# SajayR/TRIAD

Measured on AMD Instinct MI355X. Metric: tri-modal triples/sec (whole node) + loss parity, B=256 at 1/2/4/8 MI355X, higher is better.
Workload: dtype bf16

## Files before the change

### include/triad_hip.h

```cpp
#ifndef TRIAD_HIP_H
#define TRIAD_HIP_H

#include <hip/hip_runtime_api.h>

#ifdef __cplusplus
extern "C" {
#endif

#define TRIAD_EINVAL 1001

int triad_pairsim_nparts(int R_pad, int Bk);

int triad_pairsim_fwd(const void* Q, const void* K, int R, int R_pad, int Nq, int Bq, int Bk, int Nk_pad,
                      int Nk_eff, int D, const float* temp, float clamp_lo, int diag, int diag_off,
                      float* rowmax, int* argmax, double* nn_part, float* diagS, void* dS, long long CT,
                      double* st_part, const int* k_len, hipStream_t stream);

typedef struct triad_pairsim_problem {
  const void* Q;
  const void* K;
  int R, R_pad, Nq, Bq, Bk, Nk_pad, Nk_eff;
  const float* temp;
  float clamp_lo;
  int diag, diag_off;
  float* rowmax;
  int* argmax;
  double* nn_part;
  float* diagS;
  void* dS;
  long long CT;
  double* st_part;
  const int* k_tiles;
} triad_pairsim_problem;

int triad_pairsim_fwd_multi(const triad_pairsim_problem* problems, int n, hipStream_t stream);

int triad_pairsim_diag(const triad_pairsim_problem* problems, int n, hipStream_t stream);

int triad_clip_reduce(const float* rowmax, int R_pad, int Nq, int Bq, int Bk, const float* qmask, float* clip,
                      float* qw, hipStream_t stream);

int triad_diag_smooth(const float* diagS, int Bq, int Nq, int Nk_pad, int Nk_eff, double cnt, double* part,
                      float* g, double* dt_part, hipStream_t stream);

int triad_diag_sparsity(const float* diagS, int Bq, int Nt, int Nk_pad, int Nk_eff, float thr, double cnt,
                        double* part, float* g, double* dt_part, hipStream_t stream);

int triad_losshead(const float* clip, int B, int kind, const float* temp, const double* nn_part, int n_nn,
                   double n_el, const double* dg_part, int n_dg, double dg_cnt, float w_sparse, float* out,
                   float* dclip, float* lse_scratch, hipStream_t stream);

int triad_pairsim_dS(const void* Q, const void* K, int R, int R_pad, int Nq, int Bq, int Bk, int Nk_pad,
                     int Nk_eff, int D, const float* temp, float clamp_lo, int diag, int diag_off,
                     const int* argmax, const float* dclip, const float* qw, const float* dSdiag,
                     const float* coef, void* dS, long long CT, double* dt_part, hipStream_t stream);

int triad_dS_patch(void* dS, long long CT, int R, int R_pad, int Nq, int Bq, int Bk, int Nk_pad, int Nk_eff,
                   int diag_off, const int* argmax, const float* rowmax, const float* dclip, const float* qw,
                   float ratio_max, const float* gdiag, float ratio_diag, double* max_part, int n_max_part,
                   const float* temp, hipStream_t stream);

int triad_dS_patch_tiles(void* dS, long long CT, int R, int R_pad, int Nq, int Bq, int Bk, int Nk_pad, int Nk_eff,
                         int diag_off, const int* argmax, const float* rowmax, const float* dclip, const float* qw,
                         float ratio_max, const float* gdiag, float ratio_diag, double* max_part, int n_max_part,
                         const float* temp, const int* k_tiles, hipStream_t stream);

int triad_dtemp_finalize(const double* p0, int n0, const double* p1, int n1, const double* p2, int n2,
                         const float* temp, const float* w, int has_cal, float* out, hipStream_t stream);

int triad_tile_gemm(const void* Dt, long long CT, int dk, const void* B, int M, int nkt, const float* alpha,
                    int splits, float* slabs, void* C, hipStream_t stream);

int triad_tile_gemm_slabs(const void* Dt, long long CT, int dk, const void* B, int M, int nkt, int splits,
                          float* slabs, hipStream_t stream);

int triad_bfrag_pack16(const void* B, int nkt, int dk, void* Bp, hipStream_t stream);
int triad_tile_gemm_packed16(const void* Dt, long long CT, int dk, const void* Bp, int M, int nkt, const float* alpha,
                             int splits, float* slabs, void* C, hipStream_t stream);
int triad_tile_gemm_packed16_slabs(const void* Dt, long long CT, int dk, const void* Bp, int M, int nkt, int splits,
                                   float* slabs, hipStream_t stream);

int triad_gemm_bf16(const void* A, long long lda, int a_kcontig, const void* B, long long ldb, int b_kcontig,
                    int M, int N, int Kd, const float* alpha, void* C, long long ldc, int out_bf16,
                    hipStream_t stream);

int triad_gemm_bf16_bias(const void* A, long long lda, int a_kcontig, const void* B, long long ldb, int b_kcontig,
                         int M, int N, int Kd, const float* bias, void* C, long long ldc, hipStream_t stream);

int triad_gemm_bf16_bias_bf16(const void* A, long long lda, int a_kcontig, const void* B, long long ldb,
                              int b_kcontig, int M, int N, int Kd, const void* bias, void* C, long long ldc,
                              hipStream_t stream);

int triad_gemm_bf16_splitk(const void* A, long long lda, int a_kcontig, const void* B, long long ldb, int b_kcontig,
                           int M, int N, int Kd, int splits, const float* alpha, float* slabs, void* C,
                           int out_bf16, hipStream_t stream);

int triad_gemm_bf16_splitk_form(const void* A, long long lda, int a_kcontig, const void* B, long long ldb,
                                int b_kcontig, int M, int N, int Kd, int splits, const float* alpha, float* slabs,
                                void* C, int out_bf16, int form, hipStream_t stream);

int triad_gemm_bf16_form(const void* A, long long lda, int a_kcontig, const void* B, long long ldb, int b_kcontig,
                         int M, int N, int Kd, const float* alpha, void* C, long long ldc, int out_bf16, int form,
                         hipStream_t stream);

int triad_wpack(const void* W, int K, void* Bp, hipStream_t stream);
int triad_wpack2(const void* W1, int K1, void* Bp1, const void* W2, int K2, void* Bp2, hipStream_t stream);
int triad_rowpanel_count(long long M);
int triad_projhead_fwd(const void* h, long long M, int H, long long lda, long long n_per, long long bstride,
                       const void* W1p, const void* b1, const float* gamma, const float* beta, float eps,
                       const void* W2p, const void* b2, void* y1, void* ln, float* mean, float* rstd, void* y,
                       hipStream_t stream);
int triad_projhead_ln_fwd(const void* h, long long M, int H, long long lda, long long n_per, long long bstride,
                          const void* W1p, const void* b1, const float* gamma, const float* beta, float eps, void* y1,
                          void* ln, float* mean, float* rstd, hipStream_t stream);
int triad_rowgemm_bias(const void* A, long long M, int K, long long lda, const void* Bp, const void* bias, void* C,
                       hipStream_t stream);
int triad_projhead_ln_bwd(const void* dy, long long M, const void* W2p, const void* y1, const float* mean,
                          const float* rstd, const float* gamma, void* dy1, float* part, hipStream_t stream);

int triad_similarity_maps(const void* f1, const void* f2, int B, int N1, int N2, int D, const float* temp, float eps,
                          float* sim, hipStream_t stream);

int triad_ln_fwd(const void* y1, int M, const float* gamma, const float* beta, float eps, void* ln, float* mean,
                 float* rstd, hipStream_t stream);

int triad_ln_bwd3(const void* dln, const void* y1, const float* mean, const float* rstd, const float* gamma, int M,
                  void* dy1, float* part, int nblocks, hipStream_t stream);

int triad_colsum_splits(long long rows, int cols);
int triad_colsum(const void* X, long long rows, int cols, long long ld, float* part, float alpha, int out_bf16,
                 void* out, hipStream_t stream);

int triad_colsum_dma_splits(long long rows, int cols);
int triad_colsum_dma(const void* X, long long rows, int cols, long long ld, float* part, float alpha, int out_bf16,
                     void* out, hipStream_t stream);

int triad_sum_slabs(const float* slabs, int nslab, long long n, const float* alpha, int out_bf16, void* out,
                    hipStream_t stream);

int triad_global_znorm(const float* x, long long n, float eps, float* y, double* part, int nblocks,
                       hipStream_t stream);

int triad_grad_sumsq(const float* g, const void* chunks, int nchunks, double* out, hipStream_t stream);
int triad_adamw_step(float* p, const float* g, float* m, float* v, const void* chunks, int nchunks,
                     const float* pp, const float* scale, float beta1, float beta2, float omb1, float omb2,
                     float eps, const unsigned long long* shadow, hipStream_t stream);
int triad_gather_grads(const void* pieces, int npieces, float* g, int accumulate, hipStream_t stream);

int triad_gather_rows(const void* src, long long src_rows, const int* idx, int B, int M, int row_bytes, void* dst,
                      hipStream_t stream);

int triad_l2norm_rows(const void* x, int rows, int D, float eps, void* y, hipStream_t stream);

int triad_retrieval_maxmean_f32(const float* Q, const int* qlen, int Bq, int nq_pad, const float* K, const int* klen,
                                int Bk, int nk_pad, int D, float temp, float* sim, hipStream_t stream);

int triad_l2norm_rows_f32(const float* x, int rows, int D, float eps, float* y, hipStream_t stream);

long long triad_chgn_workspace_bytes(int B, int T, int C);
int triad_chgn_gelu_fwd(const void* x, int B, int T, int Tp, int C, const float* gamma, const float* beta,
                        float eps, float* mean, float* rstd, void* ws, void* y, hipStream_t stream);
int triad_chgn_gelu_bwd(const void* x, const void* dy, int B, int T, int Tp, int C, const float* gamma,
                        const float* beta, const float* mean, const float* rstd, void* ws, void* dx, float* dgamma,
                        float* dbeta, hipStream_t stream);

int triad_c0gn_fwd(const void* wave, long long Lp, const void* w0, int B, int T, int Tp, int C, const float* gamma,
                   const float* beta, float eps, float* mean, float* rstd, void* ws, void* out, void* y0out,
                   hipStream_t stream);

long long triad_conv0_dw_workspace_bytes(int B, int T, int C);
int triad_conv0_dw(const void* wave, long long Lp, const void* dy0, int B, int T, int Tp, int C, void* ws, float* dw0,
                   hipStream_t stream);

int triad_posconv(const void* x, const void* wt, const float* bias, void* y, int B, int T, int C, int groups,
                  int pad, hipStream_t stream);

long long triad_posconv_dw_part_bytes(int C, int groups, int splits);
int triad_posconv_dw(const void* x, const void* dy, int B, int T, int C, int groups, int pad, int splits, float* part,
                     hipStream_t stream);

int triad_attn_fwd(const void* q, long long q_sB, long long q_sN, const void* k, long long k_sB, long long k_sN,
                   const void* v, long long v_sB, long long v_sN, int B, int H, int N, int D, float scale, void* out,
                   long long out_sB, long long out_sN, float* lse, hipStream_t stream);
int triad_attn_bwd(const void* q, long long q_sB, long long q_sN, const void* k, long long k_sB, long long k_sN,
                   const void* v, long long v_sB, long long v_sN, const void* o, long long o_sB, long long o_sN,
                   const void* dout, long long do_sB, long long do_sN, const float* lse, int B, int H, int N, int D,
                   float scale, void* dq, long long dq_sB, long long dq_sN, void* dk, long long dk_sB,
                   long long dk_sN, void* dv, long long dv_sB, long long dv_sN, float* delta, hipStream_t stream);
int triad_attn_dropmask(int B, int H, int N, float p, unsigned seed, unsigned* wq, unsigned* wk, hipStream_t stream);
int triad_attn_fwd_dropout(const void* q, long long q_sB, long long q_sN, const void* k, long long k_sB,
                           long long k_sN, const void* v, long long v_sB, long long v_sN, int B, int H, int N, int D,
                           float scale, const unsigned* wq, float p, void* out, long long out_sB, long long out_sN,
                           float* lse, hipStream_t stream);
int triad_attn_bwd_dropout(const void* q, long long q_sB, long long q_sN, const void* k, long long k_sB,
                           long long k_sN, const void* v, long long v_sB, long long v_sN, const void* o,
                           long long o_sB, long long o_sN, const void* dout, long long do_sB, long long do_sN,
                           const float* lse, int B, int H, int N, int D, float scale, const unsigned* wq,
                           const unsigned* wk, float p, void* dq, long long dq_sB, long long dq_sN, void* dk,
                           long long dk_sB, long long dk_sN, void* dv, long long dv_sB, long long dv_sN, float* delta,
                           hipStream_t stream);

int triad_rows_nt(const void* X, long long ldx, int M, int K, const void* W, int J, void* out, hipStream_t stream);
int triad_lora_update(void* Y, long long ldy, int M, int O, const void* T, const void* Bs, hipStream_t stream);
int triad_lora_tn_blocks(int M);
int triad_lora_tn(const void* Y, long long ldy, int M, int O, const void* T, const void* Wt, void* dt, float alpha,
                  float* slabs, float* out, hipStream_t stream);

int triad_addln_fwd(const float* x, const void* y, const float* g, const float* w, const float* b, float eps, int M,
                    int D, float* xn, void* ln, int out_f32, float* mean, float* rstd, hipStream_t stream);
int triad_addln_bwd(const void* dln, int dln_f32, const float* dres, const float* xn, const float* mean,
                    const float* rstd, const float* w, const float* g, int M, int D, float* dx, void* dy,
                    hipStream_t stream);

int triad_dropaddln_fwd(const float* res, const void* y, const float* w, const float* b, float eps, int M, int D,
                        float p, unsigned seed, float* h, void* hb, float* mean, float* rstd, hipStream_t stream);
int triad_dropaddln_bwd_blocks(int M);
int triad_dropaddln_bwd(const float* dh, const void* dhb, const float* res, const void* y, const float* mean,
                        const float* rstd, const float* w, int M, int D, float p, unsigned seed, float* dres, void* dy,
                        float* part, hipStream_t stream);
long long triad_gelu_table_bytes(void);
int triad_gelu_table(void* table, hipStream_t stream);
int triad_geludrop_fwd(const void* u, long long n, float p, unsigned seed, const void* table, void* v,
                       hipStream_t stream);
int triad_geludrop_bwd(const void* u, const void* dv, long long n, float p, unsigned seed, const void* table, void* du,
                       hipStream_t stream);
int triad_dropout_keep(long long n, float p, unsigned seed, void* out, hipStream_t stream);

int triad_dense_nparts(long long n);
int triad_dense_rowmax(const float* S, int Bq, int Bk, int Nq, int Nk, int R_pad, float* rowmax, int* argmax,
                       hipStream_t stream);
int triad_nonneg_fwd(const float* S, long long n, float lo, double* part, hipStream_t stream);
int triad_nonneg_bwd(const float* S, long long n, float lo, float scale, const float* coef, float* dS,
                     hipStream_t stream);
int triad_sims_bwd_pack(const float* S, const float* dtok, const float* dclip, const float* qw, const int* argmax,
                        int Bq, int Bk, int Nq, int Nk, int R_pad, const float* temp, void* A, long long lda,
                        double* part, hipStream_t stream);
int triad_sum_parts(const double* part, int n, double scale, float* out, hipStream_t stream);

#ifdef __cplusplus
}
#endif
#endif
```

### triad_amd/_lib.py

```python
from __future__ import annotations

import ctypes as C
import os
import threading

_HERE = os.path.dirname(os.path.abspath(__file__))
DEFAULT_LIB = os.path.join(_HERE, "libtriad_hip.so")
LIB_PATH = os.environ.get("TRIAD_LIB_VARIANT", DEFAULT_LIB)

vp, i32, u32, i64, f32, f64 = C.c_void_p, C.c_int, C.c_uint, C.c_longlong, C.c_float, C.c_double

SIGNATURES = {
    "triad_pairsim_nparts": [i32, i32],
    "triad_pairsim_fwd": [vp, vp, i32, i32, i32, i32, i32, i32, i32, i32, vp, f32, i32, i32, vp, vp, vp, vp, vp,
                          i64, vp, vp, vp],
    "triad_pairsim_fwd_multi": [vp, i32, vp],
    "triad_pairsim_diag": [vp, i32, vp],
    "triad_clip_reduce": [vp, i32, i32, i32, i32, vp, vp, vp, vp],
    "triad_diag_smooth": [vp, i32, i32, i32, i32, f64, vp, vp, vp, vp],
    "triad_diag_sparsity": [vp, i32, i32, i32, i32, f32, f64, vp, vp, vp, vp],
    "triad_losshead": [vp, i32, i32, vp, vp, i32, f64, vp, i32, f64, f32, vp, vp, vp, vp],
    "triad_pairsim_dS": [vp, vp, i32, i32, i32, i32, i32, i32, i32, i32, vp, f32, i32, i32, vp, vp, vp, vp, vp,
                         vp, i64, vp, vp],
    "triad_dS_patch": [vp, i64, i32, i32, i32, i32, i32, i32, i32, i32, vp, vp, vp, vp, f32, vp, f32, vp, i32, vp,
                       vp],
    "triad_dS_patch_tiles": [vp, i64, i32, i32, i32, i32, i32, i32, i32, i32, vp, vp, vp, vp, f32, vp, f32, vp, i32,
                             vp, vp, vp],
    "triad_dtemp_finalize": [vp, i32, vp, i32, vp, i32, vp, vp, i32, vp, vp],
    "triad_tile_gemm": [vp, i64, i32, vp, i32, i32, vp, i32, vp, vp, vp],
    "triad_tile_gemm_slabs": [vp, i64, i32, vp, i32, i32, i32, vp, vp],
    "triad_bfrag_pack16": [vp, i32, i32, vp, vp],
    "triad_tile_gemm_packed16": [vp, i64, i32, vp, i32, i32, vp, i32, vp, vp, vp],
    "triad_tile_gemm_packed16_slabs": [vp, i64, i32, vp, i32, i32, i32, vp, vp],
    "triad_gemm_bf16": [vp, i64, i32, vp, i64, i32, i32, i32, i32, vp, vp, i64, i32, vp],
    "triad_gemm_bf16_bias": [vp, i64, i32, vp, i64, i32, i32, i32, i32, vp, vp, i64, vp],
    "triad_gemm_bf16_bias_bf16": [vp, i64, i32, vp, i64, i32, i32, i32, i32, vp, vp, i64, vp],
    "triad_gemm_bf16_splitk": [vp, i64, i32, vp, i64, i32, i32, i32, i32, i32, vp, vp, vp, i32, vp],
    "triad_gemm_bf16_splitk_form": [vp, i64, i32, vp, i64, i32, i32, i32, i32, i32, vp, vp, vp, i32, i32, vp],
    "triad_wpack": [vp, i32, vp, vp],
    "triad_wpack2": [vp, i32, vp, vp, i32, vp, vp],
    "triad_projhead_fwd": [vp, i64, i32, i64, i64, i64, vp, vp, vp, vp, f32, vp, vp, vp, vp, vp, vp, vp, vp],
    "triad_similarity_maps": [vp, vp, i32, i32, i32, i32, vp, f32, vp, vp],
    "triad_rowpanel_count": [i64],
    "triad_projhead_ln_fwd": [vp, i64, i32, i64, i64, i64, vp, vp, vp, vp, f32, vp, vp, vp, vp, vp],
    "triad_rowgemm_bias": [vp, i64, i32, i64, vp, vp, vp, vp],
    "triad_projhead_ln_bwd": [vp, i64, vp, vp, vp, vp, vp, vp, vp, vp],
    "triad_ln_fwd": [vp, i32, vp, vp, f32, vp, vp, vp, vp],
    "triad_ln_bwd3": [vp, vp, vp, vp, vp, i32, vp, vp, i32, vp],
    "triad_sum_slabs": [vp, i32, i64, vp, i32, vp, vp],
    "triad_colsum_splits": [i64, i32],
    "triad_colsum": [vp, i64, i32, i64, vp, f32, i32, vp, vp],
    "triad_colsum_dma_splits": [i64, i32],
    "triad_colsum_dma": [vp, i64, i32, i64, vp, f32, i32, vp, vp],
    "triad_global_znorm": [vp, i64, f32, vp, vp, i32, vp],
    "triad_grad_sumsq": [vp, vp, i32, vp, vp],
    "triad_adamw_step": [vp, vp, vp, vp, vp, i32, vp, vp, f32, f32, f32, f32, f32, vp, vp],
    "triad_gather_grads": [vp, i32, vp, i32, vp],
    "triad_gather_rows": [vp, i64, vp, i32, i32, i32, vp, vp],
    "triad_l2norm_rows": [vp, i32, i32, f32, vp, vp],
    "triad_l2norm_rows_f32": [vp, i32, i32, f32, vp, vp],
    "triad_retrieval_maxmean_f32": [vp, vp, i32, i32, vp, vp, i32, i32, i32, f32, vp, vp],
    "triad_chgn_workspace_bytes": [i32, i32, i32],
    "triad_chgn_gelu_fwd": [vp, i32, i32, i32, i32, vp, vp, f32, vp, vp, vp, vp, vp],
    "triad_chgn_gelu_bwd": [vp, vp, i32, i32, i32, i32, vp, vp, vp, vp, vp, vp, vp, vp, vp],
    "triad_gemm_bf16_form": [vp, i64, i32, vp, i64, i32, i32, i32, i32, vp, vp, i64, i32, i32, vp],
    "triad_conv0_dw_workspace_bytes": [i32, i32, i32],
    "triad_conv0_dw": [vp, i64, vp, i32, i32, i32, i32, vp, vp, vp],
    "triad_c0gn_fwd": [vp, i64, vp, i32, i32, i32, i32, vp, vp, f32, vp, vp, vp, vp, vp, vp],
    "triad_posconv": [vp, vp, vp, vp, i32, i32, i32, i32, i32, vp],
    "triad_posconv_dw_part_bytes": [i32, i32, i32],
    "triad_posconv_dw": [vp, vp, i32, i32, i32, i32, i32, i32, vp, vp],
    "triad_rows_nt": [vp, i64, i32, i32, vp, i32, vp, vp],
    "triad_lora_update": [vp, i64, i32, i32, vp, vp, vp],
    "triad_dropaddln_fwd": [vp, vp, vp, vp, f32, i32, i32, f32, u32, vp, vp, vp, vp, vp],
    "triad_dropaddln_bwd_blocks": [i32],
    "triad_dropaddln_bwd": [vp, vp, vp, vp, vp, vp, vp, i32, i32, f32, u32, vp, vp, vp, vp],
    "triad_gelu_table_bytes": [],
    "triad_gelu_table": [vp, vp],
    "triad_geludrop_fwd": [vp, i64, f32, u32, vp, vp, vp],
    "triad_geludrop_bwd": [vp, vp, i64, f32, u32, vp, vp, vp],
    "triad_dropout_keep": [i64, f32, u32, vp, vp],
    "triad_addln_fwd": [vp, vp, vp, vp, vp, f32, i32, i32, vp, vp, i32, vp, vp, vp],
    "triad_addln_bwd": [vp, i32, vp, vp, vp, vp, vp, vp, i32, i32, vp, vp, vp],
    "triad_lora_tn_blocks": [i32],
    "triad_lora_tn": [vp, i64, i32, i32, vp, vp, vp, f32, vp, vp, vp],
    "triad_attn_dropmask": [i32, i32, i32, f32, u32, vp, vp, vp],
    "triad_attn_fwd_dropout": [vp, i64, i64, vp, i64, i64, vp, i64, i64, i32, i32, i32, i32, f32, vp, f32, vp, i64,
                               i64, vp, vp],
    "triad_attn_bwd_dropout": [vp, i64, i64, vp, i64, i64, vp, i64, i64, vp, i64, i64, vp, i64, i64, vp, i32, i32,
                               i32, i32, f32, vp, vp, f32, vp, i64, i64, vp, i64, i64, vp, i64, i64, vp, vp],
    "triad_attn_fwd": [vp, i64, i64, vp, i64, i64, vp, i64, i64, i32, i32, i32, i32, f32, vp, i64, i64, vp, vp],
    "triad_attn_bwd": [vp, i64, i64, vp, i64, i64, vp, i64, i64, vp, i64, i64, vp, i64, i64, vp, i32, i32, i32,
                       i32, f32, vp, i64, i64, vp, i64, i64, vp, i64, i64, vp, vp],
    "triad_dense_nparts": [i64],
    "triad_dense_rowmax": [vp, i32, i32, i32, i32, i32, vp, vp, vp],
    "triad_nonneg_fwd": [vp, i64, f32, vp, vp],
    "triad_nonneg_bwd": [vp, i64, f32, f32, vp, vp, vp],
    "triad_sims_bwd_pack": [vp, vp, vp, vp, vp, i32, i32, i32, i32, i32, vp, vp, i64, vp, vp],
    "triad_sum_parts": [vp, i32, f64, vp, vp],
}
RESTYPES = {"triad_pairsim_nparts": C.c_int, "triad_chgn_workspace_bytes": C.c_longlong,
            "triad_conv0_dw_workspace_bytes": C.c_longlong, "triad_gelu_table_bytes": C.c_longlong,
            "triad_posconv_dw_part_bytes": C.c_longlong,
            "triad_lora_tn_blocks": C.c_int, "triad_dropaddln_bwd_blocks": C.c_int,
            "triad_colsum_splits": C.c_int, "triad_colsum_dma_splits": C.c_int, "triad_dense_nparts": C.c_int,
            "triad_rowpanel_count": C.c_int}

BACKBONE_ENTRY_POINTS = frozenset({
    "triad_chgn_gelu_fwd", "triad_chgn_gelu_bwd", "triad_gemm_bf16_form", "triad_conv0_dw", "triad_c0gn_fwd",
    "triad_posconv", "triad_posconv_dw", "triad_gemm_bf16_splitk", "triad_rows_nt", "triad_lora_update",
    "triad_dropaddln_fwd", "triad_dropaddln_bwd", "triad_gelu_table", "triad_geludrop_fwd", "triad_geludrop_bwd",
    "triad_dropout_keep", "triad_addln_fwd", "triad_addln_bwd", "triad_lora_tn", "triad_attn_dropmask",
    "triad_attn_fwd_dropout", "triad_attn_bwd_dropout", "triad_attn_fwd", "triad_attn_bwd"})


def hot_path_entry_points():
    return tuple(n for n in SIGNATURES if n not in RESTYPES and n not in BACKBONE_ENTRY_POINTS)



class PairsimProblem(C.Structure):
    _fields_ = [("Q", vp), ("K", vp), ("R", i32), ("R_pad", i32), ("Nq", i32), ("Bq", i32), ("Bk", i32),
                ("Nk_pad", i32), ("Nk_eff", i32), ("temp", vp), ("clamp_lo", f32), ("diag", i32), ("diag_off", i32),
                ("rowmax", vp), ("argmax", vp), ("nn_part", vp), ("diagS", vp), ("dS", vp), ("CT", i64),
                ("st_part", vp), ("k_tiles", vp)]


_lock = threading.Lock()
_lib = None


class TriadError(RuntimeError):
    pass


def load():
    global _lib
    with _lock:
        if _lib is None:
            if not os.path.exists(LIB_PATH):
                raise TriadError(f"{LIB_PATH} not found: build it with `python -m triad_amd.build` "
                                 "(or __graft_entry__.build()); there is no CPU fallback")
            if LIB_PATH == DEFAULT_LIB:
                _check_fresh()
            lib = C.CDLL(LIB_PATH)
            for name, args in SIGNATURES.items():
                if LIB_PATH != DEFAULT_LIB and not hasattr(lib, name):
                    continue
                fn = getattr(lib, name)
                fn.argtypes = args
                fn.restype = RESTYPES.get(name, C.c_int)
            _lib = lib
    return _lib


def _check_fresh():
    from . import build
    stamp = DEFAULT_LIB + ".srchash"
    have = open(stamp).read().strip() if os.path.exists(stamp) else None
    if have != build.source_hash():
        raise TriadError(f"{DEFAULT_LIB} is stale (built from different sources than triad_amd/csrc + "
                         "include): rebuild with `python -m triad_amd.build`")


TIMERS = None
WATCH = None


def _isolate(name):
    spec = os.environ.get("TRIAD_ISOLATE")
    return bool(spec) and name not in RESTYPES and any(name.startswith(p) for p in spec.split(",") if p)


def call(name, *args, meta=None):
    if _isolate(name):
        import torch
        torch.cuda.synchronize()
        try:
            rc = getattr(load(), name)(*args)
        finally:
            torch.cuda.synchronize()
    elif TIMERS is not None and name in TIMERS:
        import torch
        e0, e1 = torch.cuda.Event(enable_timing=True), torch.cuda.Event(enable_timing=True)
        e0.record()
        rc = getattr(load(), name)(*args)
        e1.record()
        TIMERS[name].append((e0, e1, meta))
    else:
        rc = getattr(load(), name)(*args)
    if WATCH is not None and name not in RESTYPES:
        WATCH.note(name)
    if name not in RESTYPES and rc != 0:
        what = "invalid argument/shape" if rc == 1001 else f"hipError_t {rc}"
        raise TriadError(f"{name} failed: {what}")
    return rc


def ptr(t):
    return None if t is None else C.c_void_p(t.data_ptr())


def h2d(t, device):
    import torch
    device = torch.device(device)
    if device.type != "cuda":
        return t.to(device)
    return t.pin_memory().to(device, non_blocking=True)


def stream_ptr(device=None):
    import torch
    return C.c_void_p(torch.cuda.current_stream(device).cuda_stream)
```

### triad_amd/csrc/gemm.hip

```cpp
#include "common.h"

namespace {

constexpr int BM = 128, BN = 128, BK = 64;
constexpr int A_ELEMS = BM * BK, B_ELEMS = BK * BN;

__device__ __forceinline__ int kc_off(int m, int chunk) { return m * BK + ((chunk ^ ((m >> 1) & 7)) << 3); }
__device__ __forceinline__ int nc_off(int k, int col) {
  return k * BN + ((((col >> 3) ^ ((k & 3) << 2))) << 3) + (col & 7);
}

template <bool A_KCONTIG>
__device__ __forceinline__ void stage_a_piece(const bf16* __restrict__ A, long long lda, int m0, int k0, bf16* dst,
                                              int wave, int lane, int u) {
  const int inst = wave * 4 + u;
  if (A_KCONTIG) {
    const int m = inst * 8 + (lane >> 3), cp = lane & 7;
    const int c = cp ^ ((m >> 1) & 7);
    glds16(A + (size_t)(m0 + m) * lda + k0 + c * 8, dst + inst * 512);
  } else {
    const int k = inst * 4 + (lane >> 4), cp = lane & 15;
    const int c = cp ^ ((k & 3) << 2);
    glds16(A + (size_t)(k0 + k) * lda + m0 + c * 8, dst + inst * 512);
  }
}

template <bool A_KCONTIG>
__device__ __forceinline__ void stage_a(const bf16* __restrict__ A, long long lda, int m0, int k0, bf16* dst,
                                        int wave, int lane) {
#pragma unroll
  for (int u = 0; u < 4; ++u) stage_a_piece<A_KCONTIG>(A, lda, m0, k0, dst, wave, lane, u);
}


template <bool B_KCONTIG>
__device__ __forceinline__ void stage_b(const bf16* __restrict__ B, long long ldb, int n0, int k0, bf16* dst,
                                        int wave, int lane) {
  stage_a<B_KCONTIG>(B, ldb, n0, k0, dst, wave, lane);
}

__device__ __forceinline__ bf16x8 frag_tr(const bf16* img, int n0, int s, int lane) {
  const int g = lane >> 4, i = lane & 15, q = i >> 2, p = i & 3, hh = g >> 1;
  const int col = n0 + 16 * (g & 1) + 4 * p;
  const int k0 = 16 * s + 8 * hh + q;
  const s16x4 lo = lds_tr16(img + nc_off(k0, col));
  const s16x4 hi = lds_tr16(img + nc_off(k0 + 4, col));
  bf16x8 r;
  s16x4* rp = (s16x4*)&r;
  rp[0] = lo;
  rp[1] = hi;
  return r;
}

__device__ __forceinline__ float bias_at(const void* bias, int bias_bf16, int n) {
  if (!bias) return 0.f;
  return bias_bf16 ? (float)((const bf16*)bias)[n] : ((const float*)bias)[n];
}

__device__ __forceinline__ void tile_split(int xsplit, int& tile, int& split) {
  const int T = gridDim.x;
  if (xsplit) {
    const int L = blockIdx.y * T + blockIdx.x, c = L % 8, i = L / 8;
    tile = i % T;
    split = c + 8 * (i / T);
    return;
  }
  const int bid = blockIdx.x, q8 = T / 8, r8 = T % 8, x = bid % 8;
  tile = (x < r8 ? x * (q8 + 1) : r8 * (q8 + 1) + (x - r8) * q8) + bid / 8;
  split = blockIdx.y;
}

template <bool A_KCONTIG, bool B_KCONTIG, typename OutT>
__global__ __launch_bounds__(256, 2) void gemm_kernel(const bf16* __restrict__ A, long long lda,
                                                      const bf16* __restrict__ B, long long ldb,
                                                      int M, int N, int Kd, const float* __restrict__ alpha_p,
                                                      OutT* __restrict__ C, long long ldc, int k_per_split,
                                                      long long slab_stride, const void* __restrict__ bias, int bias_bf16, int xsplit) {
  __shared__ __attribute__((aligned(16))) bf16 lds[2 * (A_ELEMS + B_ELEMS)];
  const int lane = threadIdx.x & 63, wave = __builtin_amdgcn_readfirstlane(threadIdx.x >> 6);
  const int wm = wave >> 1, wn = wave & 1;
  const int h = lane >> 5;

  int swz, split;
  tile_split(xsplit, swz, split);
  const int ntn = N / BN;
  const int m0 = (swz / ntn) * BM, n0 = (swz % ntn) * BN;

  f32x16 acc[2][2];
#pragma unroll
  for (int a = 0; a < 2; ++a)
#pragma unroll
    for (int b = 0; b < 2; ++b) acc[a][b] = (f32x16){};

  const int kbeg = split * k_per_split;
  const int nk = min(k_per_split, Kd - kbeg) / BK;
  C += (size_t)split * slab_stride;
  if (nk > 0) {
    stage_a<A_KCONTIG>(A, lda, m0, kbeg, lds, wave, lane);
    stage_b<B_KCONTIG>(B, ldb, n0, kbeg, lds + A_ELEMS, wave, lane);
  }
  for (int kt = 0; kt < nk; ++kt) {
    lds_dma_barrier();
    bf16* const nb = lds + ((kt + 1) & 1) * (A_ELEMS + B_ELEMS);
    const bool pf = kt + 1 < nk;
    if (pf) {
      stage_a<A_KCONTIG>(A, lda, m0, kbeg + (kt + 1) * BK, nb, wave, lane);
      stage_b<B_KCONTIG>(B, ldb, n0, kbeg + (kt + 1) * BK, nb + A_ELEMS, wave, lane);
    }
    const bf16* ai = lds + (kt & 1) * (A_ELEMS + B_ELEMS);
    const bf16* bi = ai + A_ELEMS;
#pragma unroll
    for (int s = 0; s < BK / 16; ++s) {
      bf16x8 af[2], bfr[2];
#pragma unroll
      for (int t = 0; t < 2; ++t) {
        const int mrow = wm * 64 + t * 32;
        if (A_KCONTIG) {
          af[t] = *(const bf16x8*)(ai + kc_off(mrow + (lane & 31), 2 * s + h));
        } else {
          af[t] = frag_tr(ai, mrow, s, lane);
        }
        const int ncol = wn * 64 + t * 32;
        if (B_KCONTIG) {
          bfr[t] = *(const bf16x8*)(bi + kc_off(ncol + (lane & 31), 2 * s + h));
        } else {
          bfr[t] = frag_tr(bi, ncol, s, lane);
        }
      }
#pragma unroll
      for (int a = 0; a < 2; ++a)
#pragma unroll
        for (int b = 0; b < 2; ++b) {
          acc[a][b] = mfma32(af[a], bfr[b], acc[a][b]);
        }
    }
  }

  const float alpha = alpha_p ? *alpha_p : 1.f;
#pragma unroll
  for (int a = 0; a < 2; ++a)
#pragma unroll
    for (int b = 0; b < 2; ++b) {
      const int n = n0 + wn * 64 + b * 32 + (lane & 31);
      const float bn = bias_at(bias, bias_bf16, n);
#pragma unroll
      for (int v = 0; v < 16; ++v) {
        const int m = m0 + wm * 64 + a * 32 + (v & 3) + 8 * (v >> 2) + 4 * h;
        C[(size_t)m * ldc + n] = (OutT)(alpha * acc[a][b][v] + bn);
      }
    }
}

constexpr int GB_M = 256, GB_NB = 3;
constexpr int GB_A = GB_M * BK, GB_ST = GB_A + B_ELEMS;
constexpr int GB_PIECES = 6;


template <bool A_KCONTIG, bool B_KCONTIG>
__device__ __forceinline__ void gb_piece(const bf16* __restrict__ A, long long lda, const bf16* __restrict__ B,
                                         long long ldb, int m0, int n0, int k0, bf16* dst, int wave, int lane,
                                         int u) {
  if (u < 4) {
    const int inst = wave * 4 + u;
    if (A_KCONTIG) {
      const int m = inst * 8 + (lane >> 3), cp = lane & 7;
      const int c = cp ^ ((m >> 1) & 7);
      glds16(A + (size_t)(m0 + m) * lda + k0 + c * 8, dst + inst * 512);
    } else {
      const int half = inst >> 4, ii = inst & 15;
      const int k = ii * 4 + (lane >> 4), cp = lane & 15;
      const int c = cp ^ ((k & 3) << 2);
      glds16(A + (size_t)(k0 + k) * lda + m0 + half * 128 + c * 8, dst + half * (BK * 128) + ii * 512);
    }
  } else {
    const int inst = wave * 2 + (u - 4);
    bf16* bd = dst + GB_A;
    if (B_KCONTIG) {
      const int n = inst * 8 + (lane >> 3), cp = lane & 7;
      const int c = cp ^ ((n >> 1) & 7);
      glds16(B + (size_t)(n0 + n) * ldb + k0 + c * 8, bd + inst * 512);
    } else {
      const int k = inst * 4 + (lane >> 4), cp = lane & 15;
      const int c = cp ^ ((k & 3) << 2);
      glds16(B + (size_t)(k0 + k) * ldb + n0 + c * 8, bd + inst * 512);
    }
  }
}

template <bool A_KCONTIG, bool B_KCONTIG, typename OutT>
__global__ __launch_bounds__(512, 1) void gemm_big_kernel(const bf16* __restrict__ A, long long lda,
                                                          const bf16* __restrict__ B, long long ldb, int M, int N,
                                                          int Kd, const float* __restrict__ alpha_p,
                                                          OutT* __restrict__ C, long long ldc, int k_per_split,
                                                          long long slab_stride, const void* __restrict__ bias, int bias_bf16, int xsplit) {
  __shared__ __attribute__((aligned(16))) bf16 lds[GB_NB * GB_ST];
  const int lane = threadIdx.x & 63, wave = __builtin_amdgcn_readfirstlane(threadIdx.x >> 6);
  const int wm = wave >> 1, wn = wave & 1;
  const int h = lane >> 5;
  int swz, split;
  tile_split(xsplit, swz, split);
  const int ntn = N / BN;
  const int m0 = (swz / ntn) * GB_M, n0 = (swz % ntn) * BN;

  f32x16 acc[2][2];
#pragma unroll
  for (int a = 0; a < 2; ++a)
#pragma unroll
    for (int b = 0; b < 2; ++b) acc[a][b] = (f32x16){};

  const int kbeg = split * k_per_split;
  const int nk = __builtin_amdgcn_readfirstlane(max(0, min(k_per_split, Kd - kbeg)) / BK);
  C += (size_t)split * slab_stride;
#pragma unroll
  for (int p = 0; p < GB_NB - 1; ++p)
    if (p < nk)
#pragma unroll
      for (int u = 0; u < GB_PIECES; ++u)
        gb_piece<A_KCONTIG, B_KCONTIG>(A, lda, B, ldb, m0, n0, kbeg + p * BK, lds + p * GB_ST, wave, lane, u);
  for (int kt = 0; kt < nk; ++kt) {
    if (kt + 1 < nk) TRIAD_VMCNT(GB_PIECES);
    else asm volatile("s_waitcnt vmcnt(0)" ::: "memory");
    __syncthreads();
    const bool pf = kt + GB_NB - 1 < nk;
    bf16* const nb = lds + ((kt + GB_NB - 1) % GB_NB) * GB_ST;
    const int kn = kbeg + (kt + GB_NB - 1) * BK;
    const bf16* ai = lds + (kt % GB_NB) * GB_ST;
    const bf16* bi = ai + GB_A;
#pragma unroll
    for (int s = 0; s < BK / 16; ++s) {
      bf16x8 af[2], bfr[2];
#pragma unroll
      for (int t = 0; t < 2; ++t) {
        const int mrow = wm * 64 + t * 32;
        if (A_KCONTIG) af[t] = *(const bf16x8*)(ai + kc_off(mrow + (lane & 31), 2 * s + h));
        else af[t] = frag_tr(ai + (mrow >> 7) * (BK * 128), mrow & 127, s, lane);
        const int ncol = wn * 64 + t * 32;
        if (B_KCONTIG) bfr[t] = *(const bf16x8*)(bi + kc_off(ncol + (lane & 31), 2 * s + h));
        else bfr[t] = frag_tr(bi, ncol, s, lane);
      }
#pragma unroll
      for (int a = 0; a < 2; ++a)
#pragma unroll
        for (int b = 0; b < 2; ++b) {
          acc[a][b] = mfma32(af[a], bfr[b], acc[a][b]);
          const int mi = s * 4 + a * 2 + b;
          if ((mi & 1) && mi / 2 < GB_PIECES) {
            __builtin_amdgcn_sched_barrier(0);
            if (pf) gb_piece<A_KCONTIG, B_KCONTIG>(A, lda, B, ldb, m0, n0, kn, nb, wave, lane, mi / 2);
            __builtin_amdgcn_sched_barrier(0);
          }
        }
    }
  }

  const float alpha = alpha_p ? *alpha_p : 1.f;
#pragma unroll
  for (int a = 0; a < 2; ++a)
#pragma unroll
    for (int b = 0; b < 2; ++b) {
      const int n = n0 + wn * 64 + b * 32 + (lane & 31);
      const float bn = bias_at(bias, bias_bf16, n);
#pragma unroll
      for (int v = 0; v < 16; ++v) {
        const int m = m0 + wm * 64 + a * 32 + (v & 3) + 8 * (v >> 2) + 4 * h;
        C[(size_t)m * ldc + n] = (OutT)(alpha * acc[a][b][v] + bn);
      }
    }
}

constexpr int GW_M = 256, GW_N = 256;
constexpr int GW_A = GW_M * BK, GW_ST = GW_A + GW_N * BK;

template <bool KCONTIG>
__device__ __forceinline__ void gw_piece_one(const bf16* __restrict__ X, long long ld, int r0, int k0, bf16* img,
                                             int inst, int lane) {
  if (KCONTIG) {
    const int m = inst * 8 + (lane >> 3), cp = lane & 7;
    const int c = cp ^ ((m >> 1) & 7);
    glds16(X + (size_t)(r0 + m) * ld + k0 + c * 8, img + inst * 512);
  } else {
    const int half = inst >> 4, ii = inst & 15;
    const int k = ii * 4 + (lane >> 4), cp = lane & 15;
    const int c = cp ^ ((k & 3) << 2);
    glds16(X + (size_t)(k0 + k) * ld + r0 + half * 128 + c * 8, img + half * (BK * 128) + ii * 512);
  }
}

template <bool KCONTIG>
__device__ __forceinline__ bf16x8 gw_frag(const bf16* img, int row, int s, int lane) {
  if (KCONTIG) return *(const bf16x8*)(img + kc_off(row + (lane & 31), 2 * s + (lane >> 5)));
  return frag_tr(img + (row >> 7) * (BK * 128), row & 127, s, lane);
}

constexpr int GE_PIECES = 8;

template <bool A_KCONTIG, bool B_KCONTIG>
__device__ __forceinline__ void ge_piece(const bf16* __restrict__ A, long long lda, const bf16* __restrict__ B,
                                         long long ldb, int m0, int n0, int k0, bf16* dst, int wave, int lane,
                                         int u) {
  if (u < 4) gw_piece_one<A_KCONTIG>(A, lda, m0, k0, dst, wave * 4 + u, lane);
  else gw_piece_one<B_KCONTIG>(B, ldb, n0, k0, dst + GW_A, wave * 4 + (u - 4), lane);
}

template <bool A_KCONTIG, bool B_KCONTIG, typename OutT>
__global__ __launch_bounds__(512, 1) void gemm_w8_kernel(const bf16* __restrict__ A, long long lda,
                                                         const bf16* __restrict__ B, long long ldb, int M, int N,
                                                         int Kd, const float* __restrict__ alpha_p,
                                                         OutT* __restrict__ C, long long ldc, int k_per_split,
                                                         long long slab_stride, const void* __restrict__ bias, int bias_bf16, int xsplit) {
  __shared__ __attribute__((aligned(16))) bf16 lds[2 * GW_ST];
  const int lane = threadIdx.x & 63, wave = __builtin_amdgcn_readfirstlane(threadIdx.x >> 6);
  const int wm = wave >> 2, wn = wave & 3;
  const int h = lane >> 5;
  int swz, split;
  tile_split(xsplit, swz, split);
  const int ntn = N / GW_N;
  const int m0 = (swz / ntn) * GW_M, n0 = (swz % ntn) * GW_N;

  f32x16 acc[4][2];
#pragma unroll
  for (int a = 0; a < 4; ++a)
#pragma unroll
    for (int b = 0; b < 2; ++b) acc[a][b] = (f32x16){};

  const int kbeg = split * k_per_split;
  const int nk = __builtin_amdgcn_readfirstlane(max(0, min(k_per_split, Kd - kbeg)) / BK);
  C += (size_t)split * slab_stride;
  if (nk > 0)
#pragma unroll
    for (int u = 0; u < GE_PIECES; ++u)
      ge_piece<A_KCONTIG, B_KCONTIG>(A, lda, B, ldb, m0, n0, kbeg, lds, wave, lane, u);
  for (int kt = 0; kt < nk; ++kt) {
    asm volatile("s_waitcnt vmcnt(0)" ::: "memory");
    __syncthreads();
    const bool pf = kt + 1 < nk;
    bf16* const nb = lds + ((kt + 1) & 1) * GW_ST;
    const int kn = kbeg + (kt + 1) * BK;
    const bf16* ai = lds + (kt & 1) * GW_ST;
    const bf16* bi = ai + GW_A;
    bf16x8 af[2][4], bfr[2][2];
#pragma unroll
    for (int t = 0; t < 4; ++t) af[0][t] = gw_frag<A_KCONTIG>(ai, wm * 128 + t * 32, 0, lane);
#pragma unroll
    for (int t = 0; t < 2; ++t) bfr[0][t] = gw_frag<B_KCONTIG>(bi, wn * 64 + t * 32, 0, lane);
#pragma unroll
    for (int s = 0; s < BK / 16; ++s) {
      const int cur = s & 1;
#pragma unroll
      for (int a = 0; a < 4; ++a)
#pragma unroll
        for (int b = 0; b < 2; ++b) {
          acc[a][b] = mfma32(af[cur][a], bfr[cur][b], acc[a][b]);
          const int j = a * 2 + b, mi = s * 8 + j;
          if (s + 1 < BK / 16 && j < 6) {
            __builtin_amdgcn_sched_barrier(0);
            if (j < 4) af[cur ^ 1][j] = gw_frag<A_KCONTIG>(ai, wm * 128 + j * 32, s + 1, lane);
            else bfr[cur ^ 1][j - 4] = gw_frag<B_KCONTIG>(bi, wn * 64 + (j - 4) * 32, s + 1, lane);
            __builtin_amdgcn_sched_barrier(0);
          }
          if (mi % 2 == 1 && mi / 2 < GE_PIECES) {
            __builtin_amdgcn_sched_barrier(0);
            if (pf) ge_piece<A_KCONTIG, B_KCONTIG>(A, lda, B, ldb, m0, n0, kn, nb, wave, lane, mi / 2);
            __builtin_amdgcn_sched_barrier(0);
          }
        }
    }
  }

  const float alpha = alpha_p ? *alpha_p : 1.f;
#pragma unroll
  for (int a = 0; a < 4; ++a)
#pragma unroll
    for (int b = 0; b < 2; ++b) {
      const int n = n0 + wn * 64 + b * 32 + (lane & 31);
      const float bn = bias_at(bias, bias_bf16, n);
#pragma unroll
      for (int v = 0; v < 16; ++v) {
        const int m = m0 + wm * 128 + a * 32 + (v & 3) + 8 * (v >> 2) + 4 * h;
        C[(size_t)m * ldc + n] = (OutT)(alpha * acc[a][b][v] + bn);
      }
    }
}


constexpr int kBigForm = 4;
constexpr int kXcdSplit = 8;


template <bool AK, bool BK_, typename OutT>
int launch(const void* A, long long lda, const void* B, long long ldb, int M, int N, int Kd, const float* alpha,
           void* C, long long ldc, hipStream_t st, int splits = 1, long long slab_stride = 0,
           const void* bias = nullptr, int form = 0, int bias_bf16 = 0) {
  const int xsplit = (form & kXcdSplit) ? 1 : 0;
  form &= ~kXcdSplit;
  if (M % BM || N % BN || Kd % BK || lda % 8 || ldb % 8 || splits < 1) return TRIAD_EINVAL;
  if (xsplit && splits % 8) return TRIAD_EINVAL;
  const int kps = ((Kd / BK + splits - 1) / splits) * BK;
  const bool w4_ok = M % GW_M == 0 && N % GW_N == 0;
  const bool w4_auto = AK && BK_ && splits == 1 && M >= 65536 && Kd >= 1024;
  if (form == 0 && w4_ok && w4_auto) form = kBigForm;
  if (w4_ok && (form == 4 || form == 3)) {
    const int nwg = (M / GW_M) * (N / GW_N);
    hipLaunchKernelGGL((gemm_w8_kernel<AK, BK_, OutT>), dim3(nwg, splits), dim3(512), 0, st, (const bf16*)A, lda,
                       (const bf16*)B, ldb, M, N, Kd, alpha, (OutT*)C, ldc, kps, slab_stride, bias, bias_bf16, xsplit);
    TRIAD_CHECK_LAUNCH();
    return TRIAD_OK;
  }
  if (form != 1 && M % GB_M == 0 &&
      (form == 2 || M >= 8192 || Kd / splits >= 32768)) {
    const int nwg = (M / GB_M) * (N / BN);
    hipLaunchKernelGGL((gemm_big_kernel<AK, BK_, OutT>), dim3(nwg, splits), dim3(512), 0, st, (const bf16*)A, lda,
                       (const bf16*)B, ldb, M, N, Kd, alpha, (OutT*)C, ldc, kps, slab_stride, bias, bias_bf16, xsplit);
    TRIAD_CHECK_LAUNCH();
    return TRIAD_OK;
  }
  const int nwg = (M / BM) * (N / BN);
  hipLaunchKernelGGL((gemm_kernel<AK, BK_, OutT>), dim3(nwg, splits), dim3(256), 0, st, (const bf16*)A, lda,
                     (const bf16*)B, ldb, M, N, Kd, alpha, (OutT*)C, ldc, kps, slab_stride, bias, bias_bf16, xsplit);
  TRIAD_CHECK_LAUNCH();
  return TRIAD_OK;
}

}

extern "C" {

int triad_gemm_bf16_form(const void* A, long long lda, int a_kcontig, const void* B, long long ldb, int b_kcontig,
                         int M, int N, int Kd, const float* alpha, void* C, long long ldc, int out_bf16, int form,
                         hipStream_t stream) {
  if (form < 0 || form > 4) return TRIAD_EINVAL;
#define TRIAD_GEMM_CASE(AK, BKC)                                                                  \
  if (!!a_kcontig == AK && !!b_kcontig == BKC)                                                   \
    return out_bf16 ? launch<AK, BKC, bf16>(A, lda, B, ldb, M, N, Kd, alpha, C, ldc, stream, 1, 0, nullptr, form) \
                    : launch<AK, BKC, float>(A, lda, B, ldb, M, N, Kd, alpha, C, ldc, stream, 1, 0, nullptr, form);
  TRIAD_GEMM_CASE(true, true)
  TRIAD_GEMM_CASE(true, false)
  TRIAD_GEMM_CASE(false, true)
  TRIAD_GEMM_CASE(false, false)
#undef TRIAD_GEMM_CASE
  return TRIAD_EINVAL;
}

int triad_gemm_bf16(const void* A, long long lda, int a_kcontig, const void* B, long long ldb, int b_kcontig,
                    int M, int N, int Kd, const float* alpha, void* C, long long ldc, int out_bf16,
                    hipStream_t stream) {
  return triad_gemm_bf16_form(A, lda, a_kcontig, B, ldb, b_kcontig, M, N, Kd, alpha, C, ldc, out_bf16, 0, stream);
}

static int gemm_bias_launch(const void* A, long long lda, int a_kcontig, const void* B, long long ldb, int b_kcontig, int M,
                     int N, int Kd, const void* bias, int bias_bf16, void* C, long long ldc, hipStream_t stream) {
  int form = 1;
  if (M >= 32768 && M % GW_M == 0 && N % GW_N == 0) form = kBigForm;
  else if (M >= 8192 && M % GB_M == 0 && (long long)(M / GB_M) * (N / BN) >= 256) form = 2;
#define TRIAD_GEMM_B(AK, BKC)                                                                     \
  if (!!a_kcontig == AK && !!b_kcontig == BKC)                                                    \
    return launch<AK, BKC, bf16>(A, lda, B, ldb, M, N, Kd, nullptr, C, ldc, stream, 1, 0, bias, form, bias_bf16);
  TRIAD_GEMM_B(true, true)
  TRIAD_GEMM_B(true, false)
  TRIAD_GEMM_B(false, true)
  TRIAD_GEMM_B(false, false)
#undef TRIAD_GEMM_B
  return TRIAD_EINVAL;
}

int triad_gemm_bf16_bias(const void* A, long long lda, int a_kcontig, const void* B, long long ldb, int b_kcontig,
                         int M, int N, int Kd, const float* bias, void* C, long long ldc, hipStream_t stream) {
  return gemm_bias_launch(A, lda, a_kcontig, B, ldb, b_kcontig, M, N, Kd, bias, 0, C, ldc, stream);
}

int triad_gemm_bf16_bias_bf16(const void* A, long long lda, int a_kcontig, const void* B, long long ldb,
                              int b_kcontig, int M, int N, int Kd, const void* bias, void* C, long long ldc,
                              hipStream_t stream) {
  return gemm_bias_launch(A, lda, a_kcontig, B, ldb, b_kcontig, M, N, Kd, bias, 1, C, ldc, stream);
}

int triad_gemm_bf16_splitk_form(const void* A, long long lda, int a_kcontig, const void* B, long long ldb,
                                int b_kcontig, int M, int N, int Kd, int splits, const float* alpha, float* slabs,
                                void* C, int out_bf16, int form, hipStream_t stream) {
  if ((form & ~kXcdSplit) < 0 || (form & ~kXcdSplit) > 4) return TRIAD_EINVAL;
  const long long slab = (long long)M * N;
  int rc = TRIAD_EINVAL;
#define TRIAD_GEMM_SK(AK, BKC)                                                                  \
  if (!!a_kcontig == AK && !!b_kcontig == BKC)                                                 \
    rc = launch<AK, BKC, float>(A, lda, B, ldb, M, N, Kd, nullptr, slabs, N, stream, splits, slab, nullptr, form);
  TRIAD_GEMM_SK(true, true)
  TRIAD_GEMM_SK(true, false)
  TRIAD_GEMM_SK(false, true)
  TRIAD_GEMM_SK(false, false)
#undef TRIAD_GEMM_SK
  if (rc) return rc;
  return triad_sum_slabs(slabs, splits, slab, alpha, out_bf16, C, stream);
}

int triad_gemm_bf16_splitk(const void* A, long long lda, int a_kcontig, const void* B, long long ldb, int b_kcontig,
                           int M, int N, int Kd, int splits, const float* alpha, float* slabs, void* C,
                           int out_bf16, hipStream_t stream) {
  return triad_gemm_bf16_splitk_form(A, lda, a_kcontig, B, ldb, b_kcontig, M, N, Kd, splits, alpha, slabs, C,
                                     out_bf16, 0, stream);
}

}
```

### triad_amd/gemm.py

```python
from __future__ import annotations

import torch
import torch.nn.functional as F

from ._lib import call, ptr, stream_ptr

_BF = torch.bfloat16
def _ok(M, N, K):
    return M > 0 and M % 128 == 0 and N % 128 == 0 and K % 64 == 0


def _rows(x):
    x2 = x.reshape(-1, x.shape[-1])
    if x2.stride(1) != 1 or x2.stride(0) != x2.shape[1]:
        x2 = x2.contiguous()
    return x2


def linear(x: torch.Tensor, w: torch.Tensor, b: torch.Tensor | None = None, meta=None) -> torch.Tensor:
    xb = x if x.dtype == _BF else x.to(_BF)
    wb = w if w.dtype == _BF else w.to(_BF)
    K = xb.shape[-1]
    N = wb.shape[0]
    x2 = _rows(xb)
    M = x2.shape[0]
    if not (x2.is_cuda and _ok(M, N, K)):
        return F.linear(xb, wb, None if b is None else b.to(_BF))
    wc = wb if wb.is_contiguous() else wb.contiguous()
    bias = None if b is None else b.detach().to(_BF).contiguous()
    out = torch.empty(M, N, dtype=_BF, device=x2.device)
    call("triad_gemm_bf16_bias_bf16", ptr(x2), K, 1, ptr(wc), K, 1, M, N, K, ptr(bias), ptr(out), N,
         stream_ptr(x2.device), meta=meta or dict(backbone=True, flops=2.0 * M * N * K))
    return out.view(*xb.shape[:-1], N)


def mm(a: torch.Tensor, b: torch.Tensor, meta=None) -> torch.Tensor:
    ab = a if a.dtype == _BF else a.to(_BF)
    bb = b if b.dtype == _BF else b.to(_BF)
    M, K = ab.shape
    N = bb.shape[1]
    if not (ab.is_cuda and _ok(M, N, K)):
        return ab @ bb
    a2 = ab if ab.is_contiguous() else ab.contiguous()
    b2 = bb if bb.is_contiguous() else bb.contiguous()
    out = torch.empty(M, N, dtype=_BF, device=a2.device)
    call("triad_gemm_bf16_bias", ptr(a2), K, 1, ptr(b2), N, 0, M, N, K, None, ptr(out), N, stream_ptr(a2.device),
         meta=meta or dict(backbone=True, flops=2.0 * M * N * K))
    return out
```

### triad_amd/linear.py

```python
from __future__ import annotations

import os

import torch
import torch.nn as nn
import torch.nn.functional as F

from . import _lib
from . import gemm as hipgemm
from ._lib import call, ptr, stream_ptr



_SPLITS_LONG = {36: 7, 108: 9, 144: 7}
_SPLITS_SHORT = {36: 7, 108: 4, 144: 3}


def _splits(M, out_f, in_f):
    tiles = (out_f // 128) * (in_f // 128)
    table = _SPLITS_LONG if M >= 32768 else _SPLITS_SHORT if 4096 <= M < 16384 else {}
    if tiles in table:
        return table[tiles]
    return min(8 if tiles <= 160 else 4, max(2, M // 2048))


_W8_SPLITS = {27: 8, 9: 24, 36: 12}
_W8_XCD = {27, 9}


def _form_splits(M, out_f, in_f):
    tiles8 = (out_f // 256) * (in_f // 256) if out_f % 256 == 0 and in_f % 256 == 0 else 0
    if M >= 32768 and tiles8 in _W8_SPLITS:
        return 4 | (8 if tiles8 in _W8_XCD else 0), _W8_SPLITS[tiles8]
    return 0, _splits(M, out_f, in_f)


def weight_grad(dy2: torch.Tensor, x2: torch.Tensor) -> torch.Tensor:
    M, O = dy2.shape
    K = x2.shape[1]
    if M % 64:
        Mp = (M + 63) // 64 * 64
        dy2 = torch.cat([dy2, dy2.new_zeros(Mp - M, O)])
        x2 = torch.cat([x2, x2.new_zeros(Mp - M, K)])
        M = Mp
    form, sp = _form_splits(M, O, K)
    slabs = torch.empty(sp * O * K, dtype=torch.float32, device=dy2.device)
    dw = torch.empty(O, K, dtype=torch.bfloat16, device=dy2.device)
    call("triad_gemm_bf16_splitk_form", ptr(dy2), dy2.stride(0), 0, ptr(x2), x2.stride(0), 0, O, K, M, sp, None,
         ptr(slabs), ptr(dw), 1, form, stream_ptr(dy2.device), meta=dict(backbone=True))
    return dw


_SIDE = {}
_JOIN_TASK = {}


def _dev_index(dev) -> int:
    dev = torch.device(dev)
    return dev.index if dev.index is not None else torch.cuda.current_device()


def _side_stream(dev):
    i = _dev_index(dev)
    s = _SIDE.get(i)
    if s is None:
        s = _SIDE[i] = torch.cuda.Stream(device=i)
    return s


def _join(dev):
    def cb():
        torch.cuda.current_stream(dev).wait_stream(_side_stream(dev))
    return cb


_CLAIMED = {}


def side_stream_ok(*ws: torch.Tensor) -> bool:
    task = torch._C._current_graph_task_id()
    if not (SIDE_STREAM_DW and task != -1 and all(w.is_cuda and w.dtype == torch.bfloat16 and w.grad is None
                                                   for w in ws)):
        return False
    dev = ws[0].device
    di = _dev_index(dev)
    t, seen = _CLAIMED.get(di, (None, None))
    if t != task:
        seen = set()
        _CLAIMED[di] = (task, seen)
    if any(id(w) in seen for w in ws):
        if di in _SIDE:
            torch.cuda.current_stream(dev).wait_stream(_SIDE[di])
        seen.update(id(w) for w in ws)
        return False
    seen.update(id(w) for w in ws)
    return True


def on_side_stream(fn, inputs):
    dev = inputs[0].device
    main = torch.cuda.current_stream(dev)
    side = _side_stream(dev)
    side.wait_stream(main)
    with torch.cuda.stream(side):
        outs = fn()
    for t in inputs:
        t.record_stream(side)
    for o in (outs if isinstance(outs, (list, tuple)) else (outs,)):
        o.record_stream(main)
    task = torch._C._current_graph_task_id()
    if _JOIN_TASK.get(_dev_index(dev)) != task:
        _JOIN_TASK[_dev_index(dev)] = task
        torch.autograd.Variable._execution_engine.queue_callback(_join(dev))
    return outs


SIDE_STREAM_DW = os.environ.get("TRIAD_SIDE_STREAM_DW", "1") != "0"


class _LinearFn(torch.autograd.Function):
    @staticmethod
    def forward(ctx, x, w, b):
        xb = x.to(torch.bfloat16)
        wb = w.to(torch.bfloat16)
        bb = None if b is None else b.to(torch.bfloat16)
        ctx.save_for_backward(xb, wb)
        ctx.meta = (x.dtype, w.dtype, None if b is None else b.dtype)
        ctx.w_ref = w
        return hipgemm.linear(xb, wb, bb)

    @staticmethod
    def backward(ctx, dy):
        xb, wb = ctx.saved_tensors
        x_dtype, w_dtype, b_dtype = ctx.meta
        O, K = wb.shape
        dy2 = dy.reshape(-1, O).to(torch.bfloat16).contiguous()
        x2 = xb.reshape(-1, K)
        if x2.stride(1) != 1 or x2.stride(0) != K:
            x2 = x2.contiguous()
        dx = dw = db = None
        if ctx.needs_input_grad[0]:
            dx = hipgemm.mm(dy2, wb).view(*xb.shape).to(x_dtype)
        if ctx.needs_input_grad[1]:
            if w_dtype == torch.bfloat16 and side_stream_ok(ctx.w_ref):
                dw = on_side_stream(lambda: weight_grad(dy2, x2), (dy2, x2))
            else:
                dw = weight_grad(dy2, x2).to(w_dtype)
        if b_dtype is not None and ctx.needs_input_grad[2]:
            from .ops import bias_grad
            db = bias_grad(dy2, torch.bfloat16 if b_dtype == torch.bfloat16 else torch.float32).to(b_dtype)
        return dx, dw, db


class _QKVFn(torch.autograd.Function):

    @staticmethod
    def forward(ctx, x, wq, bq, wk, bk, wv, bv):
        xb = x.to(torch.bfloat16)
        wb = torch.cat([wq, wk, wv]).to(torch.bfloat16)
        bb = None if bq is None else torch.cat([bq, bk, bv]).to(torch.bfloat16)
        ctx.save_for_backward(xb, wb)
        ctx.meta = (x.dtype, wq.dtype, None if bq is None else bq.dtype, (wq.shape[0], wk.shape[0], wv.shape[0]))
        ctx.w_refs = (wq, wk, wv)
        return hipgemm.linear(xb, wb, bb)

    @staticmethod
    def backward(ctx, dy):
        xb, wb = ctx.saved_tensors
        x_dtype, w_dtype, b_dtype, sizes = ctx.meta
        O, K = wb.shape
        dy2 = dy.reshape(-1, O).to(torch.bfloat16).contiguous()
        x2 = xb.reshape(-1, K)
        if x2.stride(1) != 1 or x2.stride(0) != K:
            x2 = x2.contiguous()
        dx = hipgemm.mm(dy2, wb).view(*xb.shape).to(x_dtype) if ctx.needs_input_grad[0] else None
        dws = [None] * 3
        if any(ctx.needs_input_grad[i] for i in (1, 3, 5)):
            if w_dtype == torch.bfloat16 and side_stream_ok(*ctx.w_refs):
                dws = list(on_side_stream(lambda: _split_rows(weight_grad(dy2, x2), sizes), (dy2, x2)))
            else:
                dws = [t.to(w_dtype) for t in weight_grad(dy2, x2).split(sizes)]
        dbs = [None] * 3
        if b_dtype is not None and any(ctx.needs_input_grad[i] for i in (2, 4, 6)):
            from .ops import bias_grad
            db = bias_grad(dy2, torch.bfloat16 if b_dtype == torch.bfloat16 else torch.float32).to(b_dtype)
            dbs = list(db.split(sizes))
        return dx, dws[0], dbs[0], dws[1], dbs[1], dws[2], dbs[2]


def _split_rows(buf: torch.Tensor, sizes):
    out, r = [], 0
    K = buf.shape[1]
    for n in sizes:
        t = torch.empty((0,), dtype=buf.dtype, device=buf.device)
        t.set_(buf.untyped_storage(), buf.storage_offset() + r * K, (n, K), (K, 1))
        out.append(t)
        r += n
    return out


def qkv_eligible(q: nn.Linear, k: nn.Linear, v: nn.Linear, x: torch.Tensor) -> bool:
    return (all(_eligible(m, x) for m in (q, k, v)) and q.in_features == k.in_features == v.in_features
            and (q.bias is None) == (k.bias is None) == (v.bias is None))


def qkv_projection(q: nn.Linear, k: nn.Linear, v: nn.Linear, x: torch.Tensor) -> torch.Tensor:
    return _QKVFn.apply(x, q.weight, q.bias, k.weight, k.bias, v.weight, v.bias)


def _eligible(mod: nn.Linear, x: torch.Tensor) -> bool:
    if not (x.is_cuda and torch.is_autocast_enabled("cuda") and torch.get_autocast_dtype("cuda") == torch.bfloat16):
        return False
    return x.numel() > 0 and mod.in_features % 128 == 0 and mod.out_features % 128 == 0


class TriadLinear(nn.Linear):

    def forward(self, x):
        if _eligible(self, x):
            return _LinearFn.apply(x, self.weight, self.bias)
        return super().forward(x)


def install_fast_linear(root: nn.Module) -> nn.Module:
    for mod in root.modules():
        if type(mod) is nn.Linear:
            mod.__class__ = TriadLinear
    return root
```

### triad_amd/vit.py

```python
from __future__ import annotations

import math

import torch
import torch.nn as nn
import torch.nn.functional as F

from . import attention
from . import gemm as hipgemm
from ._lib import call, ptr, stream_ptr
from .frontend import patch_embed
from .postln import gelu

ARCHS = {
    "dinov2_vits14_reg": (384, 12, 6),
    "dinov2_vitb14_reg": (768, 12, 12),
    "dinov2_vitl14_reg": (1024, 24, 16),
    "dinov2_vits14": (384, 12, 6),
    "dinov2_vitb14": (768, 12, 12),
    "dinov2_vitl14": (1024, 24, 16),
}


class _LoRALinear(torch.autograd.Function):

    @staticmethod
    def forward(ctx, x, w, b, A, B, scaling):
        lead, K = x.shape[:-1], x.shape[-1]
        O, r = B.shape
        xb = x.reshape(-1, K).to(torch.bfloat16).contiguous()
        M = xb.shape[0]
        dev = x.device
        st = stream_ptr(dev)
        Ab = A.detach().to(torch.bfloat16).contiguous()
        sB = (B.detach() * scaling).to(torch.bfloat16).contiguous()
        y = hipgemm.linear(xb, w.to(torch.bfloat16), None if b is None else b.to(torch.bfloat16)).contiguous()
        t = torch.empty(M, r, dtype=torch.bfloat16, device=dev)
        call("triad_rows_nt", ptr(xb), K, M, K, ptr(Ab), r, ptr(t), st)
        call("triad_lora_update", ptr(y), O, M, O, ptr(t), ptr(sB), st)
        ctx.save_for_backward(xb, w, Ab, sB, t)
        ctx.meta = (lead, x.dtype, float(scaling), A.dtype, B.dtype)
        return y.view(*lead, O)

    @staticmethod
    def backward(ctx, dy):
        xb, w, Ab, sB, t = ctx.saved_tensors
        lead, x_dtype, scaling, a_dtype, b_dtype = ctx.meta
        M, K = xb.shape
        O, r = sB.shape
        dev = xb.device
        dy2 = dy.reshape(M, O).to(torch.bfloat16).contiguous()
        st = stream_ptr(dev)
        dt = torch.empty(M, r, dtype=torch.bfloat16, device=dev)
        G = call("triad_lora_tn_blocks", M)
        slabs = torch.empty(G * max(O, K) * r, dtype=torch.float32, device=dev)
        wt = torch.zeros(16, O, dtype=torch.bfloat16, device=dev)
        wt[:r].copy_(sB.t())
        dB = torch.empty(O, r, dtype=torch.float32, device=dev)
        call("triad_lora_tn", ptr(dy2), O, M, O, ptr(t), ptr(wt), ptr(dt), scaling, ptr(slabs), ptr(dB), st)
        dx = None
        if ctx.needs_input_grad[0]:
            dx = hipgemm.mm(dy2, w.to(torch.bfloat16))
            At = Ab.t().contiguous()
            call("triad_lora_update", ptr(dx), K, M, K, ptr(dt), ptr(At), st)
            dx = dx.view(*lead, K).to(x_dtype)
        dAt = torch.empty(K, r, dtype=torch.float32, device=dev)
        call("triad_lora_tn", ptr(xb), K, M, K, ptr(dt), None, None, 1.0, ptr(slabs), ptr(dAt), st)
        return dx, None, None, dAt.t().to(a_dtype), dB.to(b_dtype), None


def lora_linear(x, w, b, A, B, scaling):
    return _LoRALinear.apply(x, w, b, A, B, scaling)


class LoRALinear(nn.Module):

    def __init__(self, base: nn.Linear, r: int = 8, alpha: int = 16):
        super().__init__()
        self.base = base
        self.lora_A = nn.Parameter(torch.empty(r, base.in_features))
        self.lora_B = nn.Parameter(torch.zeros(base.out_features, r))
        nn.init.kaiming_uniform_(self.lora_A, a=math.sqrt(5))
        self.scaling = alpha / r

    @property
    def weight(self):
        return self.base.weight

    def forward(self, x):
        if x.is_cuda and torch.is_autocast_enabled("cuda") and not self.base.weight.requires_grad \
                and (self.base.bias is None or not self.base.bias.requires_grad) and self.lora_A.shape[0] == 8 \
                and self.lora_A.shape[1] % 256 == 0 and self.lora_B.shape[0] % 256 == 0:
            return lora_linear(x, self.base.weight, self.base.bias, self.lora_A, self.lora_B, self.scaling)
        return self.base(x) + F.linear(F.linear(x, self.lora_A), self.lora_B) * self.scaling


class Attention(nn.Module):
    def __init__(self, dim, heads):
        super().__init__()
        self.heads = heads
        self.qkv = nn.Linear(dim, 3 * dim, bias=True)
        self.proj = nn.Linear(dim, dim, bias=True)

    def forward(self, x):
        B, N, C = x.shape
        qkv = self.qkv(x)
        if attention.supported(qkv, N, C // self.heads):
            return self.proj(attention.attention_qkv(qkv, self.heads))
        qkv = qkv.reshape(B, N, 3, self.heads, C // self.heads).permute(2, 0, 3, 1, 4)
        o = F.scaled_dot_product_attention(qkv[0], qkv[1], qkv[2])
        return self.proj(o.transpose(1, 2).reshape(B, N, C))


class LayerScale(nn.Module):
    def __init__(self, dim, init=1e-5):
        super().__init__()
        self.gamma = nn.Parameter(torch.full((dim,), init))

    def forward(self, x):
        return x * self.gamma


class Mlp(nn.Module):
    def __init__(self, dim, hidden):
        super().__init__()
        self.fc1 = nn.Linear(dim, hidden)
        self.fc2 = nn.Linear(hidden, dim)

    def forward(self, x):
        return self.fc2(gelu(self.fc1(x)))


class _AddScaleLN(torch.autograd.Function):

    @staticmethod
    def forward(ctx, x, y, g, w, b, eps, out_f32):
        M, D = x.numel() // x.shape[-1], x.shape[-1]
        dev = x.device
        if not (x.dtype == torch.float32 and y.dtype == torch.bfloat16 and y.shape == x.shape
                and all(p.dtype == torch.float32 and p.numel() == D for p in (g, w, b))):
            raise TypeError(f"add_scale_ln: x {x.dtype} {tuple(x.shape)}, y {y.dtype} {tuple(y.shape)}")
        x = x.contiguous()
        y = y.contiguous()
        xn = torch.empty_like(x)
        ln = torch.empty(x.shape, dtype=torch.float32 if out_f32 else torch.bfloat16, device=dev)
        mean = torch.empty(M, dtype=torch.float32, device=dev)
        rstd = torch.empty(M, dtype=torch.float32, device=dev)
        call("triad_addln_fwd", ptr(x), ptr(y), ptr(g), ptr(w), ptr(b), eps, M, D, ptr(xn), ptr(ln), int(out_f32),
             ptr(mean), ptr(rstd), stream_ptr(dev))
        ctx.save_for_backward(xn, mean, rstd, w, g)
        return xn, ln

    @staticmethod
    def backward(ctx, dxn, dln):
        xn, mean, rstd, w, g = ctx.saved_tensors
        M, D = xn.numel() // xn.shape[-1], xn.shape[-1]
        dev = xn.device
        if dln is None:
            dln = torch.zeros_like(xn)
        dln = dln.contiguous()
        if dln.shape != xn.shape or dln.dtype not in (torch.float32, torch.bfloat16) or \
                (dxn is not None and (dxn.shape != xn.shape or dxn.dtype != torch.float32)):
            raise TypeError("add_scale_ln backward: unexpected gradient layout")
        dxn = None if dxn is None else dxn.contiguous()
        dx = torch.empty_like(xn)
        dy = torch.empty(xn.shape, dtype=torch.bfloat16, device=dev)
        call("triad_addln_bwd", ptr(dln), int(dln.dtype == torch.float32), ptr(dxn), ptr(xn), ptr(mean), ptr(rstd),
             ptr(w), ptr(g), M, D, ptr(dx), ptr(dy), stream_ptr(dev))
        return dx, dy, None, None, None, None, None


def add_scale_ln(x, y, ls, norm, out_f32=False):
    return _AddScaleLN.apply(x, y, ls.gamma, norm.weight, norm.bias, norm.eps, out_f32)


class Block(nn.Module):
    def __init__(self, dim, heads, mlp_ratio=4.0, ls_init=1e-5):
        super().__init__()
        self.norm1 = nn.LayerNorm(dim, eps=1e-6)
        self.attn = Attention(dim, heads)
        self.ls1 = LayerScale(dim, ls_init)
        self.norm2 = nn.LayerNorm(dim, eps=1e-6)
        self.mlp = Mlp(dim, int(dim * mlp_ratio))
        self.ls2 = LayerScale(dim, ls_init)

    def forward(self, x):
        x = x + self.ls1(self.attn(self.norm1(x)))
        return x + self.ls2(self.mlp(self.norm2(x)))


class PatchEmbed(nn.Module):
    def __init__(self, patch, dim):
        super().__init__()
        self.proj = nn.Conv2d(3, dim, kernel_size=patch, stride=patch)

    def forward(self, x):
        return patch_embed(x, self.proj.weight, self.proj.bias, self.proj.stride[0])


class DinoVisionTransformer(nn.Module):

    def __init__(self, arch="dinov2_vitb14_reg", img_size=518, patch=14):
        super().__init__()
        dim, depth, heads = ARCHS[arch]
        self.embed_dim = dim
        self.patch_size = patch
        self.num_register_tokens = 4 if arch.endswith("_reg") else 0
        self.interpolate_antialias = self.num_register_tokens > 0
        self.interpolate_offset = 0.0 if self.num_register_tokens > 0 else 0.1
        grid = img_size // patch
        self.patch_embed = PatchEmbed(patch, dim)
        self.cls_token = nn.Parameter(torch.zeros(1, 1, dim))
        self.pos_embed = nn.Parameter(torch.zeros(1, 1 + grid * grid, dim))
        self.register_tokens = (nn.Parameter(torch.zeros(1, self.num_register_tokens, dim))
                                if self.num_register_tokens else None)
        self.mask_token = nn.Parameter(torch.zeros(1, dim))
        self.blocks = nn.ModuleList([Block(dim, heads) for _ in range(depth)])
        self.norm = nn.LayerNorm(dim, eps=1e-6)
        nn.init.trunc_normal_(self.pos_embed, std=0.02)
        nn.init.normal_(self.cls_token, std=1e-6)
        if self.register_tokens is not None:
            nn.init.normal_(self.register_tokens, std=1e-6)
        self.apply(self._init)
        self._pos_cache = {}

    @staticmethod
    def _init(m):
        if isinstance(m, nn.Linear):
            nn.init.trunc_normal_(m.weight, std=0.02)
            if m.bias is not None:
                nn.init.zeros_(m.bias)

    def refresh_frozen_copies(self):
        self._pos_cache = {}

    def interpolate_pos_encoding(self, n_patches_h, n_patches_w, dtype):
        key = (n_patches_h, n_patches_w, dtype, self.pos_embed._version)
        if not self.pos_embed.requires_grad and key in self._pos_cache:
            return self._pos_cache[key]
        pos = self.pos_embed.float()
        cls_pos, patch_pos = pos[:, :1], pos[:, 1:]
        M = int(math.sqrt(patch_pos.shape[1]))
        if (n_patches_h, n_patches_w) != (M, M):
            patch_pos = F.interpolate(patch_pos.reshape(1, M, M, -1).permute(0, 3, 1, 2),
                                      size=(n_patches_h, n_patches_w), mode="bicubic",
                                      antialias=self.interpolate_antialias)
            patch_pos = patch_pos.permute(0, 2, 3, 1).reshape(1, -1, pos.shape[-1])
        out = torch.cat([cls_pos, patch_pos], dim=1).to(dtype)
        if not self.pos_embed.requires_grad:
            self._pos_cache = {key: out.detach()}
        return out

    def prepare_tokens(self, x):
        B, _, H, W = x.shape
        t = self.patch_embed(x)
        t = torch.cat([self.cls_token.expand(B, -1, -1).to(t.dtype), t], dim=1)
        t = t + self.interpolate_pos_encoding(H // self.patch_size, W // self.patch_size, t.dtype)
        if self.register_tokens is not None:
            t = torch.cat([t[:, :1], self.register_tokens.expand(B, -1, -1).to(t.dtype), t[:, 1:]], dim=1)
        return t

    def _fused_ok(self, t, n, norm):
        return (t.is_cuda and n == 1 and norm and torch.is_autocast_enabled("cuda")
                and torch.get_autocast_dtype("cuda") == torch.bfloat16 and self.embed_dim % 256 == 0
                and self.embed_dim <= 1536
                and not any(p.requires_grad for blk in self.blocks
                            for m in (blk.norm1, blk.norm2, blk.ls1, blk.ls2) for p in m.parameters())
                and not any(p.requires_grad for p in self.norm.parameters()))

    def _blocks_fused(self, t):
        t = t.float()
        ln = F.layer_norm(t, (self.embed_dim,), self.blocks[0].norm1.weight, self.blocks[0].norm1.bias,
                          self.blocks[0].norm1.eps)
        last = len(self.blocks) - 1
        for i, blk in enumerate(self.blocks):
            t, ln = add_scale_ln(t, blk.attn(ln), blk.ls1, blk.norm2)
            nxt = self.norm if i == last else self.blocks[i + 1].norm1
            t, ln = add_scale_ln(t, blk.mlp(ln), blk.ls2, nxt, out_f32=i == last)
        return ln

    def get_intermediate_layers(self, x, n=1, norm=True):
        t = self.prepare_tokens(x)
        if self._fused_ok(t, n, norm):
            return (self._blocks_fused(t)[:, 1 + self.num_register_tokens:],)
        outs = []
        start = len(self.blocks) - n
        for i, blk in enumerate(self.blocks):
            t = blk(t)
            if i >= start:
                outs.append(t)
        if norm:
            outs = [self.norm(o) for o in outs]
        skip = 1 + self.num_register_tokens
        return tuple(o[:, skip:] for o in outs)

    def forward(self, x):
        t = self.prepare_tokens(x)
        for blk in self.blocks:
            t = blk(t)
        return self.norm(t)[:, 0]


def apply_lora(vit: DinoVisionTransformer, r=8, alpha=16, targets=("attn.qkv", "attn.proj")):
    for p in vit.parameters():
        p.requires_grad = False
    for blk in vit.blocks:
        if "attn.qkv" in targets:
            blk.attn.qkv = LoRALinear(blk.attn.qkv, r, alpha)
        if "attn.proj" in targets:
            blk.attn.proj = LoRALinear(blk.attn.proj, r, alpha)
    for n, p in vit.named_parameters():
        p.requires_grad = "lora_" in n
    return vit


def store_frozen_base_bf16(vit: nn.Module):
    masters = {}
    for mname, mod in vit.named_modules():
        if isinstance(mod, (nn.Linear, nn.Conv2d)):
            for pname, p in mod.named_parameters(recurse=False):
                if not p.requires_grad and p.dtype != torch.bfloat16:
                    masters[f"{mname}.{pname}" if mname else pname] = p.data.detach().to("cpu", torch.float32,
                                                                                            copy=True)
                    p.data = p.data.to(torch.bfloat16)
    vit.frozen_fp32 = {**getattr(vit, "frozen_fp32", {}), **masters}
    return vit
```

Measured before the change: 1964.

## Fuse LoRA rank-8 update into GEMM tail and bias grad into weight-grad GEMM

```diff
diff --git a/include/triad_hip.h b/include/triad_hip.h
--- a/include/triad_hip.h
+++ b/include/triad_hip.h
@@ -96,6 +96,14 @@
                            int out_bf16, hipStream_t stream);
 
 int triad_gemm_bf16_splitk_form(const void* A, long long lda, int a_kcontig, const void* B, long long ldb,
+                                int b_kcontig, int M, int N, int Kd, int splits, const float* alpha, float* slabs,
+                                void* C, int out_bf16, int form, hipStream_t stream);
+
+int triad_gemm_bf16_bias_rank8(const void* A, long long lda, int a_kcontig, const void* B, long long ldb,
+                               int b_kcontig, int M, int N, int Kd, const void* T, const void* U, const void* bias,
+                               void* C, long long ldc, int form, hipStream_t stream);
+
+int triad_gemm_bf16_splitk_bias(const void* A, long long lda, int a_kcontig, const void* B, long long ldb,
                                 int b_kcontig, int M, int N, int Kd, int splits, const float* alpha, float* slabs,
                                 void* C, int out_bf16, int form, hipStream_t stream);
 
diff --git a/triad_amd/_lib.py b/triad_amd/_lib.py
--- a/triad_amd/_lib.py
+++ b/triad_amd/_lib.py
@@ -37,6 +37,8 @@
     "triad_gemm_bf16_bias_bf16": [vp, i64, i32, vp, i64, i32, i32, i32, i32, vp, vp, i64, vp],
     "triad_gemm_bf16_splitk": [vp, i64, i32, vp, i64, i32, i32, i32, i32, i32, vp, vp, vp, i32, vp],
     "triad_gemm_bf16_splitk_form": [vp, i64, i32, vp, i64, i32, i32, i32, i32, i32, vp, vp, vp, i32, i32, vp],
+    "triad_gemm_bf16_bias_rank8": [vp, i64, i32, vp, i64, i32, i32, i32, i32, vp, vp, vp, vp, i64, i32, vp],
+    "triad_gemm_bf16_splitk_bias": [vp, i64, i32, vp, i64, i32, i32, i32, i32, i32, vp, vp, vp, i32, i32, vp],
     "triad_wpack": [vp, i32, vp, vp],
     "triad_wpack2": [vp, i32, vp, vp, i32, vp, vp],
     "triad_projhead_fwd": [vp, i64, i32, i64, i64, i64, vp, vp, vp, vp, f32, vp, vp, vp, vp, vp, vp, vp, vp],
@@ -108,7 +110,8 @@
 
 BACKBONE_ENTRY_POINTS = frozenset({
     "triad_chgn_gelu_fwd", "triad_chgn_gelu_bwd", "triad_gemm_bf16_form", "triad_conv0_dw", "triad_c0gn_fwd",
-    "triad_posconv", "triad_posconv_dw", "triad_gemm_bf16_splitk", "triad_rows_nt", "triad_lora_update",
+    "triad_posconv", "triad_posconv_dw", "triad_gemm_bf16_splitk", "triad_gemm_bf16_splitk_bias", "triad_rows_nt",
+    "triad_lora_update",
     "triad_dropaddln_fwd", "triad_dropaddln_bwd", "triad_gelu_table", "triad_geludrop_fwd", "triad_geludrop_bwd",
     "triad_dropout_keep", "triad_addln_fwd", "triad_addln_bwd", "triad_lora_tn", "triad_attn_dropmask",
     "triad_attn_fwd_dropout", "triad_attn_bwd_dropout", "triad_attn_fwd", "triad_attn_bwd"})
@@ -143,6 +146,7 @@
                                  "(or __graft_entry__.build()); there is no CPU fallback")
             if LIB_PATH == DEFAULT_LIB:
                 _check_fresh()
+            import torch
             lib = C.CDLL(LIB_PATH)
             for name, args in SIGNATURES.items():
                 if LIB_PATH != DEFAULT_LIB and not hasattr(lib, name):
diff --git a/triad_amd/csrc/gemm.hip b/triad_amd/csrc/gemm.hip
--- a/triad_amd/csrc/gemm.hip
+++ b/triad_amd/csrc/gemm.hip
@@ -57,6 +57,20 @@
   return bias_bf16 ? (float)((const bf16*)bias)[n] : ((const float*)bias)[n];
 }
 
+__device__ __forceinline__ bf16x8 r8_load(const bf16* __restrict__ X, int row, int lane) {
+  return *(const bf16x8*)(X + (size_t)(row + (lane & 31)) * 8);
+}
+__device__ __forceinline__ bf16x8 r8_frag(bf16x8 v, int lane) { return (lane >> 5) ? (bf16x8){} : v; }
+
+typedef __bf16 bf16x2 __attribute__((ext_vector_type(2)));
+__device__ __forceinline__ float frag_ksum(bf16x8 a, float c) {
+  const bf16x2 one = {(bf16)1.f, (bf16)1.f};
+  const bf16x2* p = (const bf16x2*)&a;
+#pragma unroll
+  for (int j = 0; j < 4; ++j) c = __builtin_amdgcn_fdot2_f32_bf16(p[j], one, c, false);
+  return c;
+}
+
 __device__ __forceinline__ void tile_split(int xsplit, int& tile, int& split) {
   const int T = gridDim.x;
   if (xsplit) {
@@ -70,12 +84,13 @@
   split = blockIdx.y;
 }
 
-template <bool A_KCONTIG, bool B_KCONTIG, typename OutT>
+template <bool A_KCONTIG, bool B_KCONTIG, typename OutT, bool COLSUM = false>
 __global__ __launch_bounds__(256, 2) void gemm_kernel(const bf16* __restrict__ A, long long lda,
                                                       const bf16* __restrict__ B, long long ldb,
                                                       int M, int N, int Kd, const float* __restrict__ alpha_p,
                                                       OutT* __restrict__ C, long long ldc, int k_per_split,
-                                                      long long slab_stride, const void* __restrict__ bias, int bias_bf16, int xsplit) {
+                                                      long long slab_stride, const void* __restrict__ bias, int bias_bf16, int xsplit,
+                                                      const bf16* __restrict__ T, const bf16* __restrict__ U) {
   __shared__ __attribute__((aligned(16))) bf16 lds[2 * (A_ELEMS + B_ELEMS)];
   const int lane = threadIdx.x & 63, wave = __builtin_amdgcn_readfirstlane(threadIdx.x >> 6);
   const int wm = wave >> 1, wn = wave & 1;
@@ -95,6 +110,17 @@
   const int kbeg = split * k_per_split;
   const int nk = min(k_per_split, Kd - kbeg) / BK;
   C += (size_t)split * slab_stride;
+  bf16x8 tf[2] = {}, uf[2] = {};
+  const bool tail = !COLSUM && T;
+  if (tail) {
+#pragma unroll
+    for (int t = 0; t < 2; ++t) {
+      tf[t] = r8_load(T, m0 + wm * 64 + t * 32, lane);
+      uf[t] = r8_load(U, n0 + wn * 64 + t * 32, lane);
+    }
+  }
+  const bool do_cs = COLSUM && n0 == 0 && wn == 0;
+  float cs[2] = {0.f, 0.f};
   if (nk > 0) {
     stage_a<A_KCONTIG>(A, lda, m0, kbeg, lds, wave, lane);
     stage_b<B_KCONTIG>(B, ldb, n0, kbeg, lds + A_ELEMS, wave, lane);
@@ -127,12 +153,34 @@
           bfr[t] = frag_tr(bi, ncol, s, lane);
         }
       }
+      if constexpr (COLSUM) {
+        if (do_cs) {
+#pragma unroll
+          for (int t = 0; t < 2; ++t) cs[t] = frag_ksum(af[t], cs[t]);
+        }
+      }
 #pragma unroll
       for (int a = 0; a < 2; ++a)
 #pragma unroll
         for (int b = 0; b < 2; ++b) {
           acc[a][b] = mfma32(af[a], bfr[b], acc[a][b]);
         }
+    }
+  }
+  if (tail) {
+#pragma unroll
+    for (int a = 0; a < 2; ++a)
+#pragma unroll
+      for (int b = 0; b < 2; ++b) acc[a][b] = mfma32(r8_frag(tf[a], lane), r8_frag(uf[b], lane), acc[a][b]);
+  }
+  if constexpr (COLSUM) {
+    if (do_cs) {
+      float* csum = (float*)C + (size_t)M * N;
+#pragma unroll
+      for (int t = 0; t < 2; ++t) {
+        const float v = cs[t] + __shfl_xor(cs[t], 32);
+        if (lane < 32) csum[m0 + wm * 64 + t * 32 + lane] = v;
+      }
     }
   }
 
@@ -192,7 +240,8 @@
                                                           const bf16* __restrict__ B, long long ldb, int M, int N,
                                                           int Kd, const float* __restrict__ alpha_p,
                                                           OutT* __restrict__ C, long long ldc, int k_per_split,
-                                                          long long slab_stride, const void* __restrict__ bias, int bias_bf16, int xsplit) {
+                                                          long long slab_stride, const void* __restrict__ bias, int bias_bf16, int xsplit,
+                                                          const bf16* __restrict__ T, const bf16* __restrict__ U) {
   __shared__ __attribute__((aligned(16))) bf16 lds[GB_NB * GB_ST];
   const int lane = threadIdx.x & 63, wave = __builtin_amdgcn_readfirstlane(threadIdx.x >> 6);
   const int wm = wave >> 1, wn = wave & 1;
@@ -211,6 +260,14 @@
   const int kbeg = split * k_per_split;
   const int nk = __builtin_amdgcn_readfirstlane(max(0, min(k_per_split, Kd - kbeg)) / BK);
   C += (size_t)split * slab_stride;
+  bf16x8 tf[2] = {}, uf[2] = {};
+  if (T) {
+#pragma unroll
+    for (int t = 0; t < 2; ++t) {
+      tf[t] = r8_load(T, m0 + wm * 64 + t * 32, lane);
+      uf[t] = r8_load(U, n0 + wn * 64 + t * 32, lane);
+    }
+  }
 #pragma unroll
   for (int p = 0; p < GB_NB - 1; ++p)
     if (p < nk)
@@ -251,6 +308,12 @@
           }
         }
     }
+  }
+  if (T) {
+#pragma unroll
+    for (int a = 0; a < 2; ++a)
+#pragma unroll
+      for (int b = 0; b < 2; ++b) acc[a][b] = mfma32(r8_frag(tf[a], lane), r8_frag(uf[b], lane), acc[a][b]);
   }
 
   const float alpha = alpha_p ? *alpha_p : 1.f;
@@ -302,12 +365,13 @@
   else gw_piece_one<B_KCONTIG>(B, ldb, n0, k0, dst + GW_A, wave * 4 + (u - 4), lane);
 }
 
-template <bool A_KCONTIG, bool B_KCONTIG, typename OutT>
+template <bool A_KCONTIG, bool B_KCONTIG, typename OutT, bool COLSUM = false>
 __global__ __launch_bounds__(512, 1) void gemm_w8_kernel(const bf16* __restrict__ A, long long lda,
                                                          const bf16* __restrict__ B, long long ldb, int M, int N,
                                                          int Kd, const float* __restrict__ alpha_p,
                                                          OutT* __restrict__ C, long long ldc, int k_per_split,
-                                                         long long slab_stride, const void* __restrict__ bias, int bias_bf16, int xsplit) {
+                                                         long long slab_stride, const void* __restrict__ bias, int bias_bf16, int xsplit,
+                                                         const bf16* __restrict__ T, const bf16* __restrict__ U) {
   __shared__ __attribute__((aligned(16))) bf16 lds[2 * GW_ST];
   const int lane = threadIdx.x & 63, wave = __builtin_amdgcn_readfirstlane(threadIdx.x >> 6);
   const int wm = wave >> 2, wn = wave & 3;
@@ -326,6 +390,16 @@
   const int kbeg = split * k_per_split;
   const int nk = __builtin_amdgcn_readfirstlane(max(0, min(k_per_split, Kd - kbeg)) / BK);
   C += (size_t)split * slab_stride;
+  bf16x8 tf[4] = {}, uf[2] = {};
+  const bool tail = !COLSUM && T;
+  if (tail) {
+#pragma unroll
+    for (int t = 0; t < 4; ++t) tf[t] = r8_load(T, m0 + wm * 128 + t * 32, lane);
+#pragma unroll
+    for (int t = 0; t < 2; ++t) uf[t] = r8_load(U, n0 + wn * 64 + t * 32, lane);
+  }
+  const bool do_cs = COLSUM && n0 == 0 && wn == 0;
+  float cs[4] = {0.f, 0.f, 0.f, 0.f};
   if (nk > 0)
 #pragma unroll
     for (int u = 0; u < GE_PIECES; ++u)
@@ -351,6 +425,9 @@
 #pragma unroll
         for (int b = 0; b < 2; ++b) {
           acc[a][b] = mfma32(af[cur][a], bfr[cur][b], acc[a][b]);
+          if constexpr (COLSUM) {
+            if (b == 0 && do_cs) cs[a] = frag_ksum(af[cur][a], cs[a]);
+          }
           const int j = a * 2 + b, mi = s * 8 + j;
           if (s + 1 < BK / 16 && j < 6) {
             __builtin_amdgcn_sched_barrier(0);
@@ -366,6 +443,22 @@
         }
     }
   }
+  if (tail) {
+#pragma unroll
+    for (int a = 0; a < 4; ++a)
+#pragma unroll
+      for (int b = 0; b < 2; ++b) acc[a][b] = mfma32(r8_frag(tf[a], lane), r8_frag(uf[b], lane), acc[a][b]);
+  }
+  if constexpr (COLSUM) {
+    if (do_cs) {
+      float* csum = (float*)C + (size_t)M * N;
+#pragma unroll
+      for (int t = 0; t < 4; ++t) {
+        const float v = cs[t] + __shfl_xor(cs[t], 32);
+        if (lane < 32) csum[m0 + wm * 128 + t * 32 + lane] = v;
+      }
+    }
+  }
 
   const float alpha = alpha_p ? *alpha_p : 1.f;
 #pragma unroll
@@ -387,36 +480,48 @@
 constexpr int kXcdSplit = 8;
 
 
-template <bool AK, bool BK_, typename OutT>
+inline int bias_gemm_form(int M, int N) {
+  if (M >= 32768 && M % GW_M == 0 && N % GW_N == 0) return kBigForm;
+  if (M >= 8192 && M % GB_M == 0 && (long long)(M / GB_M) * (N / BN) >= 256) return 2;
+  return 1;
+}
+
+template <bool AK, bool BK_, typename OutT, bool COLSUM = false>
 int launch(const void* A, long long lda, const void* B, long long ldb, int M, int N, int Kd, const float* alpha,
            void* C, long long ldc, hipStream_t st, int splits = 1, long long slab_stride = 0,
-           const void* bias = nullptr, int form = 0, int bias_bf16 = 0) {
+           const void* bias = nullptr, int form = 0, int bias_bf16 = 0, const void* T = nullptr,
+           const void* U = nullptr) {
   const int xsplit = (form & kXcdSplit) ? 1 : 0;
   form &= ~kXcdSplit;
   if (M % BM || N % BN || Kd % BK || lda % 8 || ldb % 8 || splits < 1) return TRIAD_EINVAL;
   if (xsplit && splits % 8) return TRIAD_EINVAL;
+  if (!T != !U || (((uintptr_t)T | (uintptr_t)U) & 15)) return TRIAD_EINVAL;
   const int kps = ((Kd / BK + splits - 1) / splits) * BK;
   const bool w4_ok = M % GW_M == 0 && N % GW_N == 0;
   const bool w4_auto = AK && BK_ && splits == 1 && M >= 65536 && Kd >= 1024;
   if (form == 0 && w4_ok && w4_auto) form = kBigForm;
   if (w4_ok && (form == 4 || form == 3)) {
     const int nwg = (M / GW_M) * (N / GW_N);
-    hipLaunchKernelGGL((gemm_w8_kernel<AK, BK_, OutT>), dim3(nwg, splits), dim3(512), 0, st, (const bf16*)A, lda,
-                       (const bf16*)B, ldb, M, N, Kd, alpha, (OutT*)C, ldc, kps, slab_stride, bias, bias_bf16, xsplit);
+    hipLaunchKernelGGL((gemm_w8_kernel<AK, BK_, OutT, COLSUM>), dim3(nwg, splits), dim3(512), 0, st, (const bf16*)A, lda,
+                       (const bf16*)B, ldb, M, N, Kd, alpha, (OutT*)C, ldc, kps, slab_stride, bias, bias_bf16, xsplit,
+                       (const bf16*)T, (const bf16*)U);
     TRIAD_CHECK_LAUNCH();
     return TRIAD_OK;
   }
   if (form != 1 && M % GB_M == 0 &&
       (form == 2 || M >= 8192 || Kd / splits >= 32768)) {
+    if (COLSUM) return TRIAD_EINVAL;
     const int nwg = (M / GB_M) * (N / BN);
     hipLaunchKernelGGL((gemm_big_kernel<AK, BK_, OutT>), dim3(nwg, splits), dim3(512), 0, st, (const bf16*)A, lda,
-                       (const bf16*)B, ldb, M, N, Kd, alpha, (OutT*)C, ldc, kps, slab_stride, bias, bias_bf16, xsplit);
+                       (const bf16*)B, ldb, M, N, Kd, alpha, (OutT*)C, ldc, kps, slab_stride, bias, bias_bf16, xsplit,
+                       (const bf16*)T, (const bf16*)U);
     TRIAD_CHECK_LAUNCH();
     return TRIAD_OK;
   }
   const int nwg = (M / BM) * (N / BN);
-  hipLaunchKernelGGL((gemm_kernel<AK, BK_, OutT>), dim3(nwg, splits), dim3(256), 0, st, (const bf16*)A, lda,
-                     (const bf16*)B, ldb, M, N, Kd, alpha, (OutT*)C, ldc, kps, slab_stride, bias, bias_bf16, xsplit);
+  hipLaunchKernelGGL((gemm_kernel<AK, BK_, OutT, COLSUM>), dim3(nwg, splits), dim3(256), 0, st, (const bf16*)A, lda,
+                     (const bf16*)B, ldb, M, N, Kd, alpha, (OutT*)C, ldc, kps, slab_stride, bias, bias_bf16, xsplit,
+                     (const bf16*)T, (const bf16*)U);
   TRIAD_CHECK_LAUNCH();
   return TRIAD_OK;
 }
@@ -448,13 +553,12 @@
 }
 
 static int gemm_bias_launch(const void* A, long long lda, int a_kcontig, const void* B, long long ldb, int b_kcontig, int M,
-                     int N, int Kd, const void* bias, int bias_bf16, void* C, long long ldc, hipStream_t stream) {
-  int form = 1;
-  if (M >= 32768 && M % GW_M == 0 && N % GW_N == 0) form = kBigForm;
-  else if (M >= 8192 && M % GB_M == 0 && (long long)(M / GB_M) * (N / BN) >= 256) form = 2;
+                     int N, int Kd, const void* bias, int bias_bf16, void* C, long long ldc, hipStream_t stream,
+                     int form = 0, const void* T = nullptr, const void* U = nullptr) {
+  if (form == 0) form = bias_gemm_form(M, N);
 #define TRIAD_GEMM_B(AK, BKC)                                                                     \
   if (!!a_kcontig == AK && !!b_kcontig == BKC)                                                    \
-    return launch<AK, BKC, bf16>(A, lda, B, ldb, M, N, Kd, nullptr, C, ldc, stream, 1, 0, bias, form, bias_bf16);
+    return launch<AK, BKC, bf16>(A, lda, B, ldb, M, N, Kd, nullptr, C, ldc, stream, 1, 0, bias, form, bias_bf16, T, U);
   TRIAD_GEMM_B(true, true)
   TRIAD_GEMM_B(true, false)
   TRIAD_GEMM_B(false, true)
@@ -472,6 +576,13 @@
                               int b_kcontig, int M, int N, int Kd, const void* bias, void* C, long long ldc,
                               hipStream_t stream) {
   return gemm_bias_launch(A, lda, a_kcontig, B, ldb, b_kcontig, M, N, Kd, bias, 1, C, ldc, stream);
+}
+
+int triad_gemm_bf16_bias_rank8(const void* A, long long lda, int a_kcontig, const void* B, long long ldb,
+                               int b_kcontig, int M, int N, int Kd, const void* T, const void* U, const void* bias,
+                               void* C, long long ldc, int form, hipStream_t stream) {
+  if (form < 0 || form > 4) return TRIAD_EINVAL;
+  return gemm_bias_launch(A, lda, a_kcontig, B, ldb, b_kcontig, M, N, Kd, bias, 1, C, ldc, stream, form, T, U);
 }
 
 int triad_gemm_bf16_splitk_form(const void* A, long long lda, int a_kcontig, const void* B, long long ldb,
@@ -492,6 +603,19 @@
   return triad_sum_slabs(slabs, splits, slab, alpha, out_bf16, C, stream);
 }
 
+int triad_gemm_bf16_splitk_bias(const void* A, long long lda, int a_kcontig, const void* B, long long ldb,
+                                int b_kcontig, int M, int N, int Kd, int splits, const float* alpha, float* slabs,
+                                void* C, int out_bf16, int form, hipStream_t stream) {
+  const int f = form & ~kXcdSplit;
+  if (f < 0 || f > 4 || f == 2 || a_kcontig) return TRIAD_EINVAL;
+  const long long slab = (long long)M * N + M;
+  int rc = b_kcontig
+      ? launch<false, true, float, true>(A, lda, B, ldb, M, N, Kd, nullptr, slabs, N, stream, splits, slab, nullptr, form)
+      : launch<false, false, float, true>(A, lda, B, ldb, M, N, Kd, nullptr, slabs, N, stream, splits, slab, nullptr, form);
+  if (rc) return rc;
+  return triad_sum_slabs(slabs, splits, slab, alpha, out_bf16, C, stream);
+}
+
 int triad_gemm_bf16_splitk(const void* A, long long lda, int a_kcontig, const void* B, long long ldb, int b_kcontig,
                            int M, int N, int Kd, int splits, const float* alpha, float* slabs, void* C,
                            int out_bf16, hipStream_t stream) {
diff --git a/triad_amd/gemm.py b/triad_amd/gemm.py
--- a/triad_amd/gemm.py
+++ b/triad_amd/gemm.py
@@ -47,3 +47,14 @@
     call("triad_gemm_bf16_bias", ptr(a2), K, 1, ptr(b2), N, 0, M, N, K, None, ptr(out), N, stream_ptr(a2.device),
          meta=meta or dict(backbone=True, flops=2.0 * M * N * K))
     return out
+
+
+def linear_rank8(a: torch.Tensor, b: torch.Tensor, b_kcontig: int, t: torch.Tensor, u: torch.Tensor,
+                 bias: torch.Tensor | None = None, form: int = 0, meta=None) -> torch.Tensor:
+    M, K = a.shape
+    N = b.shape[0] if b_kcontig else b.shape[1]
+    out = torch.empty(M, N, dtype=_BF, device=a.device)
+    call("triad_gemm_bf16_bias_rank8", ptr(a), K, 1, ptr(b), b.stride(0), b_kcontig, M, N, K, ptr(t), ptr(u),
+         ptr(bias), ptr(out), N, form, stream_ptr(a.device),
+         meta=meta or dict(backbone=True, flops=2.0 * M * N * (K + 8)))
+    return out
diff --git a/triad_amd/linear.py b/triad_amd/linear.py
--- a/triad_amd/linear.py
+++ b/triad_amd/linear.py
@@ -35,20 +35,62 @@
     return 0, _splits(M, out_f, in_f)
 
 
-def weight_grad(dy2: torch.Tensor, x2: torch.Tensor) -> torch.Tensor:
+def _pad_tokens(dy2, x2):
     M, O = dy2.shape
     K = x2.shape[1]
     if M % 64:
         Mp = (M + 63) // 64 * 64
         dy2 = torch.cat([dy2, dy2.new_zeros(Mp - M, O)])
         x2 = torch.cat([x2, x2.new_zeros(Mp - M, K)])
-        M = Mp
+    return dy2, x2
+
+
+def weight_grad(dy2: torch.Tensor, x2: torch.Tensor) -> torch.Tensor:
+    dy2, x2 = _pad_tokens(dy2, x2)
+    M, O = dy2.shape
+    K = x2.shape[1]
     form, sp = _form_splits(M, O, K)
     slabs = torch.empty(sp * O * K, dtype=torch.float32, device=dy2.device)
     dw = torch.empty(O, K, dtype=torch.bfloat16, device=dy2.device)
     call("triad_gemm_bf16_splitk_form", ptr(dy2), dy2.stride(0), 0, ptr(x2), x2.stride(0), 0, O, K, M, sp, None,
          ptr(slabs), ptr(dw), 1, form, stream_ptr(dy2.device), meta=dict(backbone=True))
     return dw
+
+
+FUSE_BIAS_GRAD = os.environ.get("TRIAD_FUSE_BIAS_GRAD", "1") != "0"
+
+
+def _bias_fusable(M, O, K):
+    form, sp = _form_splits((M + 63) // 64 * 64, O, K)
+    f = form & 7
+    if f == 1 or (f in (3, 4) and O % 256 == 0 and K % 256 == 0):
+        return True
+    if f == 2:
+        return False
+    return not (O % 256 == 0 and (O >= 8192 or (M + 63) // 64 * 64 // sp >= 32768))
+
+
+def _carve(buf: torch.Tensor, offset: int, shape):
+    t = torch.empty((0,), dtype=buf.dtype, device=buf.device)
+    strides, n = [], 1
+    for d in reversed(shape):
+        strides.append(n)
+        n *= d
+    t.set_(buf.untyped_storage(), buf.storage_offset() + offset, tuple(shape), tuple(reversed(strides)))
+    return t
+
+
+def weight_bias_grad(dy2: torch.Tensor, x2: torch.Tensor):
+    dy2, x2 = _pad_tokens(dy2, x2)
+    M, O = dy2.shape
+    K = x2.shape[1]
+    form, sp = _form_splits(M, O, K)
+    n = O * K + O
+    slabs = torch.empty(sp * n, dtype=torch.float32, device=dy2.device)
+    buf = torch.empty(n, dtype=torch.bfloat16, device=dy2.device)
+    call("triad_gemm_bf16_splitk_bias", ptr(dy2), dy2.stride(0), 0, ptr(x2), x2.stride(0), 0, O, K, M, sp, None,
+         ptr(slabs), ptr(buf), 1, form, stream_ptr(dy2.device), meta=dict(backbone=True))
+    return _carve(buf, 0, (O, K)), _carve(buf, O * K, (O,))
 
 
 _SIDE = {}
@@ -126,7 +168,7 @@
         bb = None if b is None else b.to(torch.bfloat16)
         ctx.save_for_backward(xb, wb)
         ctx.meta = (x.dtype, w.dtype, None if b is None else b.dtype)
-        ctx.w_ref = w
+        ctx.w_ref, ctx.b_ref = w, b
         return hipgemm.linear(xb, wb, bb)
 
     @staticmethod
@@ -141,12 +183,21 @@
         dx = dw = db = None
         if ctx.needs_input_grad[0]:
             dx = hipgemm.mm(dy2, wb).view(*xb.shape).to(x_dtype)
+        want_b = b_dtype is not None and ctx.needs_input_grad[2]
+        if (FUSE_BIAS_GRAD and ctx.needs_input_grad[1] and want_b and b_dtype == torch.bfloat16
+                and _bias_fusable(dy2.shape[0], O, K)):
+            if w_dtype == torch.bfloat16 and side_stream_ok(ctx.w_ref, ctx.b_ref):
+                dw, db = on_side_stream(lambda: weight_bias_grad(dy2, x2), (dy2, x2))
+            else:
+                dw, db = weight_bias_grad(dy2, x2)
+                dw = dw.to(w_dtype)
+            return dx, dw, db
         if ctx.needs_input_grad[1]:
             if w_dtype == torch.bfloat16 and side_stream_ok(ctx.w_ref):
                 dw = on_side_stream(lambda: weight_grad(dy2, x2), (dy2, x2))
             else:
                 dw = weight_grad(dy2, x2).to(w_dtype)
-        if b_dtype is not None and ctx.needs_input_grad[2]:
+        if want_b:
             from .ops import bias_grad
             db = bias_grad(dy2, torch.bfloat16 if b_dtype == torch.bfloat16 else torch.float32).to(b_dtype)
         return dx, dw, db
@@ -161,7 +212,7 @@
         bb = None if bq is None else torch.cat([bq, bk, bv]).to(torch.bfloat16)
         ctx.save_for_backward(xb, wb)
         ctx.meta = (x.dtype, wq.dtype, None if bq is None else bq.dtype, (wq.shape[0], wk.shape[0], wv.shape[0]))
-        ctx.w_refs = (wq, wk, wv)
+        ctx.w_refs, ctx.b_refs = (wq, wk, wv), (bq, bk, bv)
         return hipgemm.linear(xb, wb, bb)
 
     @staticmethod
@@ -175,6 +226,19 @@
             x2 = x2.contiguous()
         dx = hipgemm.mm(dy2, wb).view(*xb.shape).to(x_dtype) if ctx.needs_input_grad[0] else None
         dws = [None] * 3
+        want_w = all(ctx.needs_input_grad[i] for i in (1, 3, 5))
+        want_b = b_dtype is not None and all(ctx.needs_input_grad[i] for i in (2, 4, 6))
+        if FUSE_BIAS_GRAD and want_w and want_b and b_dtype == torch.bfloat16 and _bias_fusable(dy2.shape[0], O, K):
+            def both():
+                dw, db = weight_bias_grad(dy2, x2)
+                offs = (0, sizes[0], sizes[0] + sizes[1])
+                return _split_rows(dw, sizes) + [_carve(db, o, (n,)) for o, n in zip(offs, sizes)]
+            if w_dtype == torch.bfloat16 and side_stream_ok(*ctx.w_refs, *ctx.b_refs):
+                g = list(on_side_stream(both, (dy2, x2)))
+            else:
+                g = both()
+                g[:3] = [t.to(w_dtype) for t in g[:3]]
+            return dx, g[0], g[3], g[1], g[4], g[2], g[5]
         if any(ctx.needs_input_grad[i] for i in (1, 3, 5)):
             if w_dtype == torch.bfloat16 and side_stream_ok(*ctx.w_refs):
                 dws = list(on_side_stream(lambda: _split_rows(weight_grad(dy2, x2), sizes), (dy2, x2)))
diff --git a/triad_amd/vit.py b/triad_amd/vit.py
--- a/triad_amd/vit.py
+++ b/triad_amd/vit.py
@@ -34,10 +34,15 @@
         st = stream_ptr(dev)
         Ab = A.detach().to(torch.bfloat16).contiguous()
         sB = (B.detach() * scaling).to(torch.bfloat16).contiguous()
-        y = hipgemm.linear(xb, w.to(torch.bfloat16), None if b is None else b.to(torch.bfloat16)).contiguous()
+        wb = w.to(torch.bfloat16)
+        bb = None if b is None else b.detach().to(torch.bfloat16).contiguous()
         t = torch.empty(M, r, dtype=torch.bfloat16, device=dev)
         call("triad_rows_nt", ptr(xb), K, M, K, ptr(Ab), r, ptr(t), st)
-        call("triad_lora_update", ptr(y), O, M, O, ptr(t), ptr(sB), st)
+        if hipgemm._ok(M, O, K):
+            y = hipgemm.linear_rank8(xb, wb if wb.is_contiguous() else wb.contiguous(), 1, t, sB, bb)
+        else:
+            y = hipgemm.linear(xb, wb, bb).contiguous()
+            call("triad_lora_update", ptr(y), O, M, O, ptr(t), ptr(sB), st)
         ctx.save_for_backward(xb, w, Ab, sB, t)
         ctx.meta = (lead, x.dtype, float(scaling), A.dtype, B.dtype)
         return y.view(*lead, O)
@@ -60,9 +65,13 @@
         call("triad_lora_tn", ptr(dy2), O, M, O, ptr(t), ptr(wt), ptr(dt), scaling, ptr(slabs), ptr(dB), st)
         dx = None
         if ctx.needs_input_grad[0]:
-            dx = hipgemm.mm(dy2, w.to(torch.bfloat16))
+            wb = w.to(torch.bfloat16)
             At = Ab.t().contiguous()
-            call("triad_lora_update", ptr(dx), K, M, K, ptr(dt), ptr(At), st)
+            if hipgemm._ok(M, K, O):
+                dx = hipgemm.linear_rank8(dy2, wb if wb.is_contiguous() else wb.contiguous(), 0, dt, At)
+            else:
+                dx = hipgemm.mm(dy2, wb)
+                call("triad_lora_update", ptr(dx), K, M, K, ptr(dt), ptr(At), st)
             dx = dx.view(*lead, K).to(x_dtype)
         dAt = torch.empty(K, r, dtype=torch.float32, device=dev)
         call("triad_lora_tn", ptr(xb), K, M, K, ptr(dt), None, None, 1.0, ptr(slabs), ptr(dAt), st)
```

Measured after the change: 1935. 0.985x the previous value.
